# jasonkyuyim/se3_diffusion

Measured on AMD Instinct MI355X. Metric: residues/sec IPA fwd+bwd, higher is better.
Workload: dtype f32

## Files before the change

### include/fd_hip.h

```cpp
#ifndef FD_HIP_H_
#define FD_HIP_H_

#ifdef __cplusplus
extern "C" {
#endif

#define FD_ABI_VERSION 2

const char* fd_last_error(void);
int fd_abi_version(void);
const char* fd_backend(void);
const char* fd_build_flags(void);
long fd_launch_count(void);

typedef struct FdGemmDesc {
  const float* A;
  const float* B;
  float* C;
  int M, N, K;
  long a_rs, a_cs;
  long b_rs, b_cs;
  long ldc;
  int batch, bdiv;
  long a_so, a_si, b_so, b_si, c_so, c_si;
  float alpha;
  int beta;
  const float* bias;
  const float* pair_p;
  const float* pair_q;
  long ld_pair;
  int nres;
  const float* resid;
  long ld_resid;
  const float* gate;
  long ld_gate;
  const float* rowscale;
  int relu;
  int tile;
  int ksplit;
  int mtiles;
  float* a_rowsum;
  const void* b_planes;
  long b_plane_stride;
} FdGemmDesc;

int fd_gemm(const FdGemmDesc* desc, void* stream);
int fd_split_planes(const float* x, long n, void* planes, void* stream);
int fd_gemm_plan(const FdGemmDesc* desc);
int fd_gemm_set_exact_f32(int exact);
int fd_gemm_set_persistent_blocks(int blocks);

int fd_layernorm_fwd(const float* x, long ldx, const float* gamma, const float* beta, const float* rowscale,
                     float* y, long ldy, float* mean, float* rstd, long rows, int C, float eps, void* stream);
int fd_layernorm_bwd(const float* dy, long lddy, const float* x, long ldx, const float* gamma,
                     const float* rowscale, const float* mean, const float* rstd, float* dx, long lddx,
                     int dx_accum, float* dgamma, float* dbeta, long rows, int C, void* stream);
int fd_colsum_acc(const float* X, long ld, long rows, int ncols, float* out, void* stream);
int fd_pair_reduce_acc(const float* X, int nbatch, int n, int C, float* rowsum, float* colsum, long ld_out,
                       void* stream);
int fd_axpby(float* y, const float* x, float a, float b, long n, void* stream);
int fd_add2d(float* dst, long ldd, const float* src, long lds, long rows, int cols, float a, void* stream);
int fd_rowscale(const float* x, long ldx, const float* rs, float* y, long ldy, long rows, int C, void* stream);

#define FD_EDGE_MLP_IMAGE_BYTES (124 * 12288)
int fd_edge_mlp_pack_zb(const float* W40, void* image, void* stream);
int fd_edge_mlp_pack(const float* W1, const float* W2, const float* Wf, long ld, void* image, void* stream);
int fd_edge_mlp_pack_bwd(const float* Wf, const float* W2, const float* W1, long ld, const float* W40, void* image, void* stream);
typedef struct FdEdgeMlpDesc {
  const float* x;
  const void* img;
  const float* p1;
  const float* q1;
  const float* bias2;
  float* save1;
  float* save2;
  const float* pf;
  const float* qf;
  const float* gamma;
  const float* beta;
  const float* rowscale;
  float* y;
  float* mean;
  float* rstd;
  float* out;
  long rows;
  int nres;
  int backward;
  float eps;
  int blocks;
  long ld_pq;
  long ld_pqf;
  float* zb_out;
  const float* zb_bias;
  unsigned* mask1;
  unsigned* mask2;
  const unsigned* gmask1;
  const unsigned* gmask2;
  const float* ln_y;
  const float* ln_mean;
  const float* ln_rstd;
// ... 173 lines not shown
                     float* A, int B, int N, int heads_per_block, void* stream);
#define FD_IPA_FLASH_PART_LD 328
int fd_ipa_flash_fwd_split(const float* proj, const float* zb, const float* qp, const float* kp, const float* vp,
                           const float* head_w, const float* mask, const float* quat, const float* trans, float* feats,
                           float* A, int B, int N, int heads_per_block, int key_splits, float* part, void* stream);

int fd_ipa_flash_bwd(const float* proj, const float* A, const float* zb, const float* dfeats, const float* feats,
                     const float* doptg, const float* ptdot, const float* qp, const float* kp, const float* vp,
                     const float* head_w, const float* trans, float* dL, float* dzb, float* dqp, float* dkp,
                     float* dhead_w, float* hw_part, int B, int N, void* stream);
int fd_ipa_flash_bwd_keys(const float* A, const float* dL, const float* proj, const float* dfeats, const float* doptg,
                          const float* qp, const float* kp, const float* head_w, float* dproj, float* dvp, float* dkp,
                          int B, int N, int heads_per_block, void* stream);
int fd_ipa_opt_bwd_dot(const float* dfeats, const float* feats, const float* quat, const float* trans, float* doptg,
                       float* dframe, float* ptdot, long R, void* stream);

int fd_ipa_dz_acc(const float* dzb, const float* W40, float* dz, long rows, int accumulate, void* stream);

int fd_ipa_kpts_bwd(const float* dL, const float* qp, const float* kp, const float* head_w, float* dkp, int B, int N,
                    void* stream);

int fd_row_softmax_fwd(float* S, const float* key_add, long rows, int N, int rows_per_batch, void* stream);
int fd_row_softmax_bwd(const float* A, float* dA, long rows, int N, void* stream);

int fd_split_rigids(const float* rig7, float scale, const float* t, float tscale, float* quat, float* trans, float* tscaled,
                    long R, int B, void* stream);

int fd_bb_update_fwd(const float* node, long ldn, int cs, const float* dmask, const float* W6, const float* b6,
                     const float* quat, const float* trans, float* upd, float* quat_out, float* trans_out,
                     long R, void* stream);
int fd_bb_update_bwd(const float* dquat_out, const float* dtrans_out, const float* dframe, const float* dmask,
                     const float* upd, const float* quat, float* dquat, float* dtrans, float* dupd, float* dupd_s,
                     long R, void* stream);

typedef struct FdHeadConst {
  float atoms[15];
  float Rd[9];
  float td[3];
  float coord_scale;
  double exp_max_sigma, exp_min_sigma;
  float min_b, max_b;
  int L;
  const double* score_norms;
  const double* omega_grid;
  int n_omega;
} FdHeadConst;
int fd_heads_fwd(const float* rig0, const float* quatF, const float* transF, const float* upsi,
                 const float* gt_psi, long gt_stride, const float* fixed, const float* mask, const float* t,
                 const double* sigma_grid, int ng, const FdHeadConst* c, double* rot_score, float* trans_score,
                 float* rigids, float* psi_out, float* atom37, float* atom14,
                 float* sc_ca_out ,
                 int B, int N, void* stream);
int fd_backbone_atoms(const float* rigids, const float* psi, const FdHeadConst* c, float* atom37, float* atom14,
                      long R, void* stream);
int fd_heads_bwd(const float* rig0, const float* quatF, const float* transF, const float* upsi,
                 const float* psi_out, const float* fixed, const float* mask, const float* t,
                 const double* sigma_grid, int ng, const FdHeadConst* c, const double* d_rot,
                 const float* d_trans_score, const float* d_rigids, const float* d_psi, const float* d_atom37,
                 float* dquatF, float* dtransF, float* dupsi, int B, int N, void* stream);

int fd_igso3_tables(const double* sigma, const double* omega, int ns, int no, int L, double* pdf, double* cdf,
                    double* score_norms, void* stream);
int fd_sample_ref(const double* z_axis, const double* u, const double* z_trans, const double* cdf_row,
                  const double* omega, int no, double coord_scale, float* out, long n, void* stream);
int fd_forward_marginal(const float* rig0, const double* z_axis, const double* u, const double* z_trans,
                        const double* cdf_row, const double* omega, int no,
// ... 100 lines not shown
```

### se3_diffusion_amd/csrc/fd_edge_embed.hip

```cpp
#include "fd_common.h"
#include "../../include/fd_hip.h"

namespace {

#include "fd_chain.h"

constexpr int EE_UNITS = 20;
constexpr int EE_ZB_UNITS = 4;
constexpr int EE_ZB = 40;
constexpr int EE_C = 128;
constexpr float kPi = 3.14159265358979323846f;

__global__ __launch_bounds__(256) void edge_embed_pack_kernel(const float* __restrict__ W0, const float* __restrict__ W2,
                                                              const float* __restrict__ W4, char* __restrict__ img) {
  const int gid = (int)(blockIdx.x * blockDim.x + threadIdx.x);
  if (gid >= EE_UNITS * 4 * 64) return;
  const int lane = gid & 63, i = (gid >> 6) & 3, u = gid >> 8;
  const int m = lane & 15, g = lane >> 4;
  const int layer = u < 4 ? 0 : (u < 12 ? 1 : 2);
  const int r = u - (layer == 0 ? 0 : (layer == 1 ? 4 : 12));
  const int n = 64 * (r & 1) + 16 * i + m, k0 = 32 * (r >> 1);
  float x[8];
#pragma unroll
  for (int e = 0; e < 8; ++e) {
    if (layer == 0) {
      const int k = k0 + 8 * g + e;
      x[e] = k < 54 ? W0[n * 120 + 66 + k] : 0.f;
    } else {
      const int k = k0 + 16 * (e >> 2) + 4 * g + (e & 3);
      x[e] = (layer == 1 ? W2 : W4)[n * EE_C + k];
    }
  }
  uint4 s0, s1, s2;
  em_split8(x, s0, s1, s2);
  char* dst = img + (long)u * EM_UNIT + (i * 3) * EM_PIECE + lane * 16;
  *reinterpret_cast<uint4*>(dst) = s0;
  *reinterpret_cast<uint4*>(dst + EM_PIECE) = s1;
  *reinterpret_cast<uint4*>(dst + 2 * EM_PIECE) = s2;
}

__global__ __launch_bounds__(256) void edge_embed_pack_zb_kernel(const float* __restrict__ W40, char* __restrict__ img) {
  const int gid = (int)(blockIdx.x * blockDim.x + threadIdx.x);
  if (gid >= EE_ZB_UNITS * 4 * 64) return;
  const int lane = gid & 63, i = (gid >> 6) & 3, ks = gid >> 8;
  const int m = lane & 15, g = lane >> 4;
  const int n = 16 * i + m;
  float x[8];
#pragma unroll
  for (int e = 0; e < 8; ++e) {
    const int k = 32 * ks + 16 * (e >> 2) + 4 * g + (e & 3);
    x[e] = n < EE_ZB ? W40[n * EE_C + k] : 0.f;
  }
  uint4 s0, s1, s2;
  em_split8(x, s0, s1, s2);
  char* dst = img + (long)(EE_UNITS + ks) * EM_UNIT + (i * 3) * EM_PIECE + lane * 16;
  *reinterpret_cast<uint4*>(dst) = s0;
  *reinterpret_cast<uint4*>(dst + EM_PIECE) = s1;
  *reinterpret_cast<uint4*>(dst + 2 * EM_PIECE) = s2;
}

template <bool ZB>
__global__ __launch_bounds__(64 * EM_WAVES, 2) void edge_embed_kernel(FdEdgeEmbedDesc d) {
  constexpr int EE_NSTAGE = (EE_UNITS + (ZB ? EE_ZB_UNITS : 0)) / EM_UPS;
  __shared__ __attribute__((aligned(16))) char lds[2 * EM_STAGE];
  const int tid = (int)threadIdx.x;
  const int lane = tid & 63, wave = tid >> 6;
  const int m = lane & 15, g = lane >> 4;
  const long rows = d.rows;
  const long ld_pq = d.ld_pq > 0 ? d.ld_pq : EE_C;
  const int ntiles = (int)((rows + EM_ROWS - 1) / EM_ROWS);
  const int G = (int)gridDim.x, first = (int)blockIdx.x;
  if (first >= ntiles) return;
  const int nmine = (ntiles - first + G - 1) / G;
  const int total_stages = nmine * EE_NSTAGE;

  const char* __restrict__ img_lane = static_cast<const char*>(d.img) + wave * (EM_STAGE / EM_WAVES) + lane * 16;
  char* const lds_wave = lds + wave * (EM_STAGE / EM_WAVES);
  int issued = 0, consumed = 0;
  auto issue_stage = [&]() {
    const char* src = img_lane + (long)(issued % EE_NSTAGE) * EM_STAGE;
    char* dst = lds_wave + (issued & 1) * EM_STAGE;
    fd::glds16x4(src, dst);
    fd::glds16x2(src + 4096, dst + 4096);
    ++issued;
  };
  auto stage_begin = [&]() -> const char* {
    fd::wait_vmem();
    __syncthreads();
    const char* cur = lds + (consumed & 1) * EM_STAGE + lane * 16;
    ++consumed;
    return cur;
// ... 253 lines not shown
```

### se3_diffusion_amd/csrc/fd_edge_embed_bwd.hip

```cpp
#include "fd_common.h"
#include "../../include/fd_hip.h"

namespace {

#include "fd_chain.h"

constexpr int EB_UNITS = 16;
constexpr int EB_NSTAGE = EB_UNITS / EM_UPS;
constexpr int EB_C = 128;

__global__ __launch_bounds__(256) void edge_embed_bwd_pack_kernel(const float* __restrict__ W2, const float* __restrict__ W4,
                                                                  char* __restrict__ img) {
  const int gid = (int)(blockIdx.x * blockDim.x + threadIdx.x);
  if (gid >= EB_UNITS * 4 * 64) return;
  const int lane = gid & 63, i = (gid >> 6) & 3, u = gid >> 8;
  const int m = lane & 15, g = lane >> 4;
  const int layer = u >> 3, r = u & 7;
  const int n = 64 * (r & 1) + 16 * i + m, k0 = 32 * (r >> 1);
  const float* __restrict__ W = layer == 0 ? W4 : W2;
  float x[8];
#pragma unroll
  for (int e = 0; e < 8; ++e) {
    const int k = k0 + 16 * (e >> 2) + 4 * g + (e & 3);
    x[e] = W[k * EB_C + n];
  }
  uint4 s0, s1, s2;
  em_split8(x, s0, s1, s2);
  char* dst = img + (long)u * EM_UNIT + (i * 3) * EM_PIECE + lane * 16;
  *reinterpret_cast<uint4*>(dst) = s0;
  *reinterpret_cast<uint4*>(dst + EM_PIECE) = s1;
  *reinterpret_cast<uint4*>(dst + 2 * EM_PIECE) = s2;
}

__global__ __launch_bounds__(64 * EM_WAVES, 2) void edge_embed_bwd_kernel(FdEdgeEmbedBwdDesc d) {
  __shared__ __attribute__((aligned(16))) char lds[2 * EM_STAGE];
  const int tid = (int)threadIdx.x;
  const int lane = tid & 63, wave = tid >> 6;
  const int m = lane & 15, g = lane >> 4;
  const long rows = d.rows;
  const int ntiles = (int)((rows + EM_ROWS - 1) / EM_ROWS);
  const int G = (int)gridDim.x, first = (int)blockIdx.x;
  if (first >= ntiles) return;
  unsigned* const sched = d.sched;
  const bool dyn = sched != nullptr;
  __shared__ int s_tile;
  const int nmine = (ntiles - first + G - 1) / G;
  const int total_stages = dyn ? 0x7fffffff : nmine * EB_NSTAGE;

  const char* __restrict__ img_lane = static_cast<const char*>(d.img) + wave * (EM_STAGE / EM_WAVES) + lane * 16;
  char* const lds_wave = lds + wave * (EM_STAGE / EM_WAVES);
  int issued = 0, consumed = 0;
  auto issue_stage = [&]() {
    const char* src = img_lane + (long)(issued % EB_NSTAGE) * EM_STAGE;
    char* dst = lds_wave + (issued & 1) * EM_STAGE;
    fd::glds16x4(src, dst);
    fd::glds16x2(src + 4096, dst + 4096);
    ++issued;
  };
  auto stage_begin = [&]() -> const char* {
    fd::wait_vmem();
    __syncthreads();
    const char* cur = lds + (consumed & 1) * EM_STAGE + lane * 16;
    ++consumed;
    return cur;
  };
  auto stage_prefetch = [&]() {
    if (issued < total_stages) issue_stage();
  };
  issue_stage();

  f32x4 dgam[8], dbet[8];
#pragma unroll
  for (int nb = 0; nb < 8; ++nb)
#pragma unroll
    for (int e = 0; e < 4; ++e) dgam[nb][e] = dbet[nb][e] = 0.f;

  int tile = first, nxt = 0;
  for (int ti = 0;;) {
    if (dyn && tid == 0) nxt = G + (int)atomicAdd(&sched[0], 1u);
    const long row = (long)tile * EM_ROWS + wave * 16 + m;
    const bool rok = row < rows;
    const long rc = rok ? row : rows - 1;

    const bool packed = d.gmask2 != nullptr;
    unsigned gm2 = 0u, gm1 = 0u;
    if (packed) {
      gm2 = d.gmask2[rc * 4 + g];
      gm1 = d.gmask1[rc * 4 + g];
    }

    f32x4 d3[8];
    {
      const float rs = (d.rowscale != nullptr ? d.rowscale[rc] : 1.f) * (rok ? 1.f : 0.f);
      const float mean = d.mean[rc], rstd = d.rstd[rc];
      float s1 = 0.f, s2 = 0.f;
#pragma unroll
      for (int nb = 0; nb < 8; ++nb) {
        const int col = 16 * nb + 4 * g;
        const float4 dy = *reinterpret_cast<const float4*>(d.dy + rc * EB_C + col);
        const float4 h = *reinterpret_cast<const float4*>(d.h3 + rc * EB_C + col);
        const float4 gm = *reinterpret_cast<const float4*>(d.gamma + col);
        const float dyv[4] = {dy.x, dy.y, dy.z, dy.w}, hv[4] = {h.x, h.y, h.z, h.w}, gv[4] = {gm.x, gm.y, gm.z, gm.w};
#pragma unroll
        for (int e = 0; e < 4; ++e) {
          const float x = (hv[e] - mean) * rstd;
          const float gy = dyv[e] * rs;
          dgam[nb][e] += gy * x;
          dbet[nb][e] += gy;
          const float t = gy * gv[e];
          d3[nb][e] = t;
          s1 += t;
          s2 += t * x;
// ... 132 lines not shown
    float a = 0.f;
#pragma unroll
    for (int w = 0; w < EM_WAVES; ++w) a += red[(w * 2 + which) * EB_C + col];
    float* dst = which == 0 ? d.dgamma : d.dbeta;
    if (dst != nullptr) atomicAdd(dst + col, a);
  }
}

}

extern "C" int fd_edge_embed_bwd_pack(const float* W2, const float* W4, void* img, void* stream) {
  FD_CHECK_ARG(W2 && W4 && img, "fd_edge_embed_bwd_pack: null operand");
  FD_CHECK_ARG(fd_aligned16(img), "fd_edge_embed_bwd_pack: image must be 16-byte aligned");
  hipLaunchKernelGGL(edge_embed_bwd_pack_kernel, dim3(EB_UNITS * 4 * 64 / 256), dim3(256), 0, (hipStream_t)stream, W2, W4,
                     static_cast<char*>(img));
  FD_CHECK_LAUNCH("fd_edge_embed_bwd_pack");
  return FD_OK;
}

extern "C" int fd_edge_embed_bwd(const FdEdgeEmbedBwdDesc* desc, void* stream) {
  FD_CHECK_ARG(desc != nullptr, "fd_edge_embed_bwd: null descriptor");
  const FdEdgeEmbedBwdDesc& d = *desc;
  FD_CHECK_ARG(d.dy && d.h3 && d.mean && d.rstd && d.gamma && d.img && d.dh3 && d.dh2 && d.dh1,
               "fd_edge_embed_bwd: a required operand is null");
  FD_CHECK_ARG((d.h2 && d.h1) || (d.gmask2 && d.gmask1), "fd_edge_embed_bwd: h2 / h1 or their packed sign masks are required");
  FD_CHECK_ARG(d.rows >= 0, "fd_edge_embed_bwd: negative row count");
  const void* ptrs[] = {d.dy, d.h3, d.gamma, d.h2, d.h1, d.img, d.dh3, d.dh2, d.dh1};
  for (const void* p : ptrs) FD_CHECK_ARG(fd_aligned16(p), "fd_edge_embed_bwd: operands must be 16-byte aligned");
  if (d.rows == 0) return FD_OK;
  const long ntiles = (d.rows + EM_ROWS - 1) / EM_ROWS;
  const int blocks = d.blocks > 0 ? d.blocks : 256 * EM_BLOCKS_PER_CU;
  const long grid = ntiles < blocks ? ntiles : blocks;
  FdEdgeEmbedBwdDesc dd = d;
  if (dd.sched != nullptr && ntiles >= 4 * grid) {
    FD_CHECK_ARG(hipMemsetAsync(dd.sched, 0, sizeof(unsigned), (hipStream_t)stream) == hipSuccess,
                 "fd_edge_embed_bwd: zeroing the tile counter failed");
  } else {
    dd.sched = nullptr;
  }
  hipLaunchKernelGGL(edge_embed_bwd_kernel, dim3((unsigned)grid), dim3(64 * EM_WAVES), 0, (hipStream_t)stream, dd);
  FD_CHECK_LAUNCH("fd_edge_embed_bwd");
  return FD_OK;
}
```

### se3_diffusion_amd/csrc/fd_edge_mlp.hip

```cpp
#if defined(EM_PHASE_TIMING) || defined(EM_ABLATE_PQ) || defined(EM_PLAIN_SAVES)
#include "fd_probe.h"
#endif
#include "fd_common.h"
#include "../../include/fd_hip.h"

#ifdef EM_SHAPE_W8
#define EM_LAUNCH fd_edge_mlp_launch_w8
#else
#define EM_LAUNCH fd_edge_mlp_launch_w4
#endif
int fd_edge_mlp_launch_w4(const FdEdgeMlpDesc& d, hipStream_t st);
int fd_edge_mlp_launch_w8(const FdEdgeMlpDesc& d, hipStream_t st);
int fd_edge_mlp_launch_pair(const FdEdgeMlpDesc& d, hipStream_t st);

namespace {

#include "fd_chain.h"

__device__ __forceinline__ float fd_f4(const float4& v, int e) { return e == 0 ? v.x : e == 1 ? v.y : e == 2 ? v.z : v.w; }

constexpr int EM_UNITS = 120;
constexpr int EM_ZB_UNITS = 4;
constexpr int EM_ZB = 40;
constexpr int EM_RING = 2;
constexpr int EM_H = 384, EM_C = 128;
#ifdef EM_PLAIN_SAVES
#define EM_SAVE4(p, a, b, c, e) (*reinterpret_cast<float4*>(p) = make_float4((a), (b), (c), (e)))
#else
#define EM_SAVE4(p, a, b, c, e) fd::store_nt4((p), (a), (b), (c), (e))
#endif

#ifdef EM_PHASE_TIMING
__device__ unsigned long long em_phase[12];
#define EM_TICK_TO(var)                                                \
  {                                                                    \
    __builtin_amdgcn_sched_barrier(0);                                 \
    const long long t_ = (long long)__builtin_amdgcn_s_memtime();      \
    __builtin_amdgcn_sched_barrier(0);                                 \
    var += t_ - tl_;                                                   \
    tl_ = t_;                                                          \
  }
#define EM_BODY_TO(i) { EM_TICK_TO(tb_); em_add(i, tb_); tb_ = 0; }
#else
#define EM_TICK_TO(var)
#define EM_BODY_TO(i)
#endif

#ifndef EM_SHAPE_W8
struct EmMat {
  const float* p;
  long rs, cs;
};

__global__ __launch_bounds__(256) void edge_mlp_pack16_kernel(EmMat A1, EmMat A2, EmMat A4, char* __restrict__ img, int rot) {
  const int gid = (int)(blockIdx.x * blockDim.x + threadIdx.x);
  if (gid >= EM_UNITS * 4 * 64) return;
  const int lane = gid & 63, i = (gid >> 6) & 3, u = gid >> 8;
  const int m = lane & 15, g = lane >> 4;
  EmMat M;
  int n, k0;
  if (u < 96) {
    const int c = u / 32, r = u % 32, hc = (c + rot) % 3;
    if (r < 8) {
      M = A1; n = 128 * hc + 64 * (r & 1) + 16 * i + m; k0 = 32 * (r >> 1);
    } else {
      const int r2 = r - 8;
      M = A2; n = 64 * (r2 % 6) + 16 * i + m; k0 = 128 * hc + 32 * (r2 / 6);
    }
  } else {
    const int v = u - 96;
    M = A4; n = 64 * (v & 1) + 16 * i + m; k0 = 32 * (v >> 1);
  }
  float x[8];
#pragma unroll
  for (int e = 0; e < 8; ++e) {
    const int k = k0 + 16 * (e >> 2) + 4 * g + (e & 3);
    x[e] = M.p[(long)n * M.rs + (long)k * M.cs];
  }
  uint4 s0, s1, s2;
  em_split8(x, s0, s1, s2);
  char* dst = img + (long)u * EM_UNIT + (i * 3) * EM_PIECE + lane * 16;
  *reinterpret_cast<uint4*>(dst) = s0;
  *reinterpret_cast<uint4*>(dst + EM_PIECE) = s1;
  *reinterpret_cast<uint4*>(dst + 2 * EM_PIECE) = s2;
}

__global__ __launch_bounds__(256) void edge_mlp_pack_zb_kernel(const float* __restrict__ W40, char* __restrict__ img) {
  const int gid = (int)(blockIdx.x * blockDim.x + threadIdx.x);
  if (gid >= EM_ZB_UNITS * 4 * 64) return;
  const int lane = gid & 63, i = (gid >> 6) & 3, ks = gid >> 8;
  const int m = lane & 15, g = lane >> 4;
  const int n = 16 * i + m;
  float x[8];
#pragma unroll
  for (int e = 0; e < 8; ++e) {
    const int k = 32 * ks + 16 * (e >> 2) + 4 * g + (e & 3);
    x[e] = n < EM_ZB ? W40[n * EM_C + k] : 0.f;
  }
  uint4 s0, s1, s2;
  em_split8(x, s0, s1, s2);
  char* dst = img + (long)(EM_UNITS + ks) * EM_UNIT + (i * 3) * EM_PIECE + lane * 16;
  *reinterpret_cast<uint4*>(dst) = s0;
  *reinterpret_cast<uint4*>(dst + EM_PIECE) = s1;
  *reinterpret_cast<uint4*>(dst + 2 * EM_PIECE) = s2;
}

__global__ __launch_bounds__(256) void edge_mlp_pack_zbw_kernel(const float* __restrict__ W40, char* __restrict__ img) {
  const int gid = (int)(blockIdx.x * blockDim.x + threadIdx.x);
  if (gid >= EM_ZB_UNITS * 4 * 64) return;
  const int lane = gid & 63, i = (gid >> 6) & 3, u = gid >> 8;
  const int m = lane & 15, g = lane >> 4;
  const int n = 64 * (u & 1) + 16 * i + m, k0 = 32 * (u >> 1);
  float x[8];
#pragma unroll
  for (int e = 0; e < 8; ++e) {
    const int k = k0 + 8 * g + e;
    x[e] = k < EM_ZB ? W40[k * EM_C + n] : 0.f;
  }
  uint4 s0, s1, s2;
  em_split8(x, s0, s1, s2);
  char* dst = img + (long)u * EM_UNIT + (i * 3) * EM_PIECE + lane * 16;
  *reinterpret_cast<uint4*>(dst) = s0;
  *reinterpret_cast<uint4*>(dst + EM_PIECE) = s1;
  *reinterpret_cast<uint4*>(dst + 2 * EM_PIECE) = s2;
}

#endif

template <bool BWD, bool ZB = false, bool TRAIN = false, bool LNB = false, bool ZBW = false>
__global__ __launch_bounds__(64 * EM_WAVES, 2) void edge_mlp16_kernel(FdEdgeMlpDesc d) {
  static_assert(!BWD || (!ZB && TRAIN), "backward: no zb layer, always with the saves");
  static_assert(BWD || (!LNB && !ZBW), "the fused prologue is a backward option");
  constexpr int EM_NSTAGE = (EM_UNITS + (ZB ? EM_ZB_UNITS : 0) + (ZBW ? EM_ZB_UNITS : 0)) / EM_UPS;
  __shared__ __attribute__((aligned(16))) char lds[EM_RING * EM_STAGE];
  __shared__ float lnacc[LNB ? 2 * EM_C : 1];
  const int tid = (int)threadIdx.x;
  const int lane = tid & 63, wave = tid >> 6;
  const int m = lane & 15, g = lane >> 4;
  const long rows = d.rows;
#ifdef EM_PHASE_TIMING
  long long p0_ = 0, p1_ = 0, p2_ = 0, p3_ = 0, p4_ = 0, p5_ = 0, p6_ = 0, p7_ = 0, p8_ = 0, p9_ = 0;
  long long tb_ = 0, tl_ = (long long)__builtin_amdgcn_s_memtime();
  auto em_add = [&](int i, long long v) {
    switch (i) {
      case 0: p0_ += v; break;
      case 2: p2_ += v; break;
      case 3: p3_ += v; break;
      case 4: p4_ += v; break;
      case 5: p5_ += v; break;
      case 6: p6_ += v; break;
      case 7: p7_ += v; break;
      case 8: p8_ += v; break;
      default: p9_ += v; break;
    }
  };
#endif
  const long ld_pq = d.ld_pq > 0 ? d.ld_pq : EM_H, ld_pqf = d.ld_pqf > 0 ? d.ld_pqf : EM_C;
// ... 10 lines not shown
  char* const lds_wave = lds + wave * (EM_STAGE / EM_WAVES);
  int issued = 0, consumed = 0;
  auto issue_stage = [&]() __attribute__((always_inline)) {
    const char* src = img_lane + (long)(issued % EM_NSTAGE) * EM_STAGE;
    char* dst = lds_wave + (issued % EM_RING) * EM_STAGE;
    if (EM_PPW == 6) {
      fd::glds16x4(src, dst);
      fd::glds16x2(src + 4096, dst + 4096);
    } else {
      fd::glds16x3(src, dst);
    }
    ++issued;
  };
  auto stage_begin = [&]() __attribute__((always_inline)) -> const char* {
    EM_TICK_TO(tb_);
    fd::wait_vmem();
    __syncthreads();
    EM_TICK_TO(p1_);
    const char* cur = lds + (consumed % EM_RING) * EM_STAGE + lane * 16;
    ++consumed;
    return cur;
  };
  auto stage_prefetch = [&]() __attribute__((always_inline)) {
    if (issued < total_stages) issue_stage();
  };
  issue_stage();
  if (LNB) {
    if (tid < 2 * EM_C) lnacc[tid] = 0.f;
    __syncthreads();
  }

  int tile = first, nxt = 0;
  for (int ti = 0;;) {
    if (dyn && tid == 0) nxt = G + (int)atomicAdd(&sched[0], 1u);
    const long row = (long)tile * EM_ROWS + wave * 16 + m;
    const bool rok = row < rows;
    const long rc = rok ? row : rows - 1;
    const long qi = rc / d.nres;
    const long qj = (qi / d.nres) * d.nres + (rc - qi * d.nres);

    f32x4 X[BWD ? 8 : 1], Xk[2][2];
    auto load_xk = [&](int buf, int ks) __attribute__((always_inline)) {
#pragma unroll
      for (int i = 0; i < 2; ++i) {
        const float4 v = *reinterpret_cast<const float4*>(d.x + rc * EM_C + 16 * (2 * ks + i) + 4 * g);
        Xk[buf][i][0] = v.x; Xk[buf][i][1] = v.y; Xk[buf][i][2] = v.z; Xk[buf][i][3] = v.w;
      }
    };
    if (BWD) {
#pragma unroll
      for (int nb = 0; nb < 8; ++nb) {
        float4 v = make_float4(0.f, 0.f, 0.f, 0.f);
        if (!LNB || d.x != nullptr) v = *reinterpret_cast<const float4*>(d.x + rc * EM_C + 16 * nb + 4 * g);
        X[nb][0] = v.x; X[nb][1] = v.y; X[nb][2] = v.z; X[nb][3] = v.w;
      }
    } else {
      load_xk(0, 0);
    }
    if (LNB) {
      if (ZBW) {
        float kz[2][8];
        {
          const float* zp = d.dzb + rc * EM_ZB + 8 * g;
          const float4 v = *reinterpret_cast<const float4*>(zp);
          const float4 w = *reinterpret_cast<const float4*>(zp + 4);
          kz[0][0] = v.x; kz[0][1] = v.y; kz[0][2] = v.z; kz[0][3] = v.w;
          kz[0][4] = w.x; kz[0][5] = w.y; kz[0][6] = w.z; kz[0][7] = w.w;
// ... 343 lines not shown
  }
  if (tid == 0) __hip_atomic_fetch_add(&em_phase[10], 1ull, __ATOMIC_RELAXED, __HIP_MEMORY_SCOPE_AGENT);
#endif
  if (dyn) fd::wait_vmem();
  if (LNB) {
    __syncthreads();
    if (tid < EM_C) {
      if (d.ln_dgamma != nullptr) atomicAdd(d.ln_dgamma + tid, lnacc[tid]);
    } else if (tid < 2 * EM_C) {
      if (d.ln_dbeta != nullptr) atomicAdd(d.ln_dbeta + (tid - EM_C), lnacc[tid]);
    }
  }
}

}

#ifdef EM_PHASE_TIMING
extern "C" int fd_edge_mlp_phases(unsigned long long* host12, int reset) {
  if (host12 != nullptr && hipMemcpyFromSymbol(host12, HIP_SYMBOL(em_phase), sizeof(em_phase)) != hipSuccess) return -1;
  if (reset) {
    unsigned long long z[12] = {0};
    if (hipMemcpyToSymbol(HIP_SYMBOL(em_phase), z, sizeof(z)) != hipSuccess) return -1;
  }
  return 0;
}
#endif

int EM_LAUNCH(const FdEdgeMlpDesc& d, hipStream_t st) {
  const long ntiles = (d.rows + EM_ROWS - 1) / EM_ROWS;
  const int blocks = d.blocks > 0 ? d.blocks : 256 * EM_BLOCKS_PER_CU;
  const int grid = (int)(ntiles < blocks ? ntiles : blocks);
  const dim3 g3(grid), b3(64 * EM_WAVES);
  FdEdgeMlpDesc dd = d;
  if (dd.sched != nullptr && ntiles >= 4L * grid) {
    FD_CHECK_ARG(hipMemsetAsync(dd.sched, 0, sizeof(unsigned), st) == hipSuccess, "fd_edge_mlp: zeroing the tile counter failed");
  } else {
    dd.sched = nullptr;
  }
  const bool zbv = d.zb_out != nullptr, train = d.save1 != nullptr;
#define EM_GO(...) hipLaunchKernelGGL(HIP_KERNEL_NAME(edge_mlp16_kernel<__VA_ARGS__>), g3, b3, 0, st, dd)
  if (d.backward) {
    if (d.ln_y != nullptr && d.dzb != nullptr) EM_GO(true, false, true, true, true);
    else if (d.ln_y != nullptr) EM_GO(true, false, true, true, false);
    else EM_GO(true, false, true, false, false);
  } else if (zbv) {
    if (train) EM_GO(false, true, true); else EM_GO(false, true, false);
  } else {
    if (train) EM_GO(false, false, true); else EM_GO(false, false, false);
  }
#undef EM_GO
  FD_CHECK_LAUNCH("fd_edge_mlp");
  return FD_OK;
}

#ifndef EM_SHAPE_W8
extern "C" int fd_edge_mlp_pack(const float* W1, const float* W2, const float* Wf, long ld, void* img, void* stream) {
  FD_CHECK_ARG(W1 && W2 && Wf && img, "fd_edge_mlp_pack: null operand");
  FD_CHECK_ARG(fd_aligned16(img), "fd_edge_mlp_pack: image must be 16-byte aligned");
  EmMat m1{W1, ld, 1}, m2{W2, ld, 1}, m4{Wf, ld, 1};
  hipLaunchKernelGGL(edge_mlp_pack16_kernel, dim3(EM_UNITS * 4 * 64 / 256), dim3(256), 0, (hipStream_t)stream, m1, m2, m4,
                     static_cast<char*>(img), 0);
  FD_CHECK_LAUNCH("fd_edge_mlp_pack");
  return FD_OK;
}

extern "C" int fd_edge_mlp_pack_bwd(const float* Wf, const float* W2, const float* W1, long ld, const float* W40, void* img,
                                    void* stream) {
  FD_CHECK_ARG(Wf && W2 && W1 && img, "fd_edge_mlp_pack_bwd: null operand");
  FD_CHECK_ARG(fd_aligned16(img), "fd_edge_mlp_pack_bwd: image must be 16-byte aligned");
  char* base = static_cast<char*>(img);
  if (W40 != nullptr) {
    hipLaunchKernelGGL(edge_mlp_pack_zbw_kernel, dim3(EM_ZB_UNITS * 4 * 64 / 256), dim3(256), 0, (hipStream_t)stream, W40, base);
    base += (long)EM_ZB_UNITS * EM_UNIT;
  }
  EmMat m1{Wf, 1, ld}, m2{W2, 1, ld}, m4{W1, 1, ld};
  hipLaunchKernelGGL(edge_mlp_pack16_kernel, dim3(EM_UNITS * 4 * 64 / 256), dim3(256), 0, (hipStream_t)stream, m1, m2, m4, base, 1);
  FD_CHECK_LAUNCH("fd_edge_mlp_pack_bwd");
  return FD_OK;
}

extern "C" int fd_edge_mlp_pack_zb(const float* W40, void* img, void* stream) {
  FD_CHECK_ARG(W40 && img, "fd_edge_mlp_pack_zb: null operand");
  FD_CHECK_ARG(fd_aligned16(img), "fd_edge_mlp_pack_zb: image must be 16-byte aligned");
  hipLaunchKernelGGL(edge_mlp_pack_zb_kernel, dim3(EM_ZB_UNITS * 4 * 64 / 256), dim3(256), 0, (hipStream_t)stream, W40,
                     static_cast<char*>(img));
  FD_CHECK_LAUNCH("fd_edge_mlp_pack_zb");
  return FD_OK;
}

extern "C" int fd_edge_mlp(const FdEdgeMlpDesc* desc, void* stream) {
  FD_CHECK_ARG(desc != nullptr, "fd_edge_mlp: null descriptor");
  const FdEdgeMlpDesc& d = *desc;
  FD_CHECK_ARG(d.img && d.out && (d.x || (d.backward && d.ln_y && d.dzb)), "fd_edge_mlp: x / img / out are required");
  FD_CHECK_ARG(d.ln_y == nullptr || (d.backward && d.ln_mean && d.ln_rstd && d.ln_gamma),
               "fd_edge_mlp: the fused LayerNorm backward (ln_y) is a backward option and needs ln_mean / ln_rstd / ln_gamma");
  FD_CHECK_ARG(d.dzb == nullptr || d.ln_y != nullptr, "fd_edge_mlp: dzb needs the fused LayerNorm-backward prologue (ln_y)");
  FD_CHECK_ARG(d.nres > 0 && d.rows >= 0, "fd_edge_mlp: bad extents");
  if (d.backward) {
    FD_CHECK_ARG(d.gmask1 && d.gmask2 && d.save1 && d.save2,
                 "fd_edge_mlp(backward): the packed sign masks of h2 (gmask1) and h1 (gmask2) and the outputs d2 (save1) / d1 (save2) "
                 "are required");
    FD_CHECK_ARG(!d.mask1 && !d.mask2 && !d.zb_out, "fd_edge_mlp(backward): mask1 / mask2 / zb_out are forward outputs");
  } else {
    FD_CHECK_ARG(d.p1 && d.q1 && d.bias2 && d.pf && d.qf && d.gamma && d.beta,
                 "fd_edge_mlp(forward): p1 / q1 / bias2 / pf / qf / gamma / beta are required");
    const int nsave = (d.save1 != nullptr) + (d.save2 != nullptr) + (d.mask1 != nullptr) + (d.mask2 != nullptr);
    FD_CHECK_ARG(nsave == 0 || nsave == 4,
                 "fd_edge_mlp(forward): the training outputs save1 (h1), save2 (h2 + [z | 0 | 0]), mask1, mask2 come together");
    FD_CHECK_ARG(nsave == 4 || (!d.y && !d.mean && !d.rstd), "fd_edge_mlp(forward): y / mean / rstd are training outputs (with the saves)");
    FD_CHECK_ARG(!d.gmask1 && !d.gmask2, "fd_edge_mlp(forward): gmask1 / gmask2 are backward inputs");
  }
  const void* ptrs[] = {d.x, d.img, d.out, d.p1, d.q1, d.bias2, d.save1, d.save2, d.pf, d.qf,
                        d.gamma, d.beta, d.y, d.ln_y, d.ln_gamma, d.dy_out, d.dzb};
  for (const void* p : ptrs) FD_CHECK_ARG(fd_aligned16(p), "fd_edge_mlp: operands must be 16-byte aligned");
  if (d.rows == 0) return FD_OK;
  FD_CHECK_ARG(d.zb_out == nullptr || (fd_aligned16(d.zb_out) && fd_aligned16(d.zb_bias)),
               "fd_edge_mlp: zb_out / zb_bias must be 16-byte aligned (the image must carry the fd_edge_mlp_pack_zb units)");
  FD_CHECK_ARG(d.shape == 0 || d.shape == 2 || d.shape == 4 || d.shape == 8,
               "fd_edge_mlp: shape is 0 (by size), 2 (two waves per 16 rows: inference forward), 4 or 8 (waves per block)");
// ... 10 lines not shown
```

### se3_diffusion_amd/csrc/fd_frames.hip

```cpp
#include "fd_common.h"
#include "../../include/fd_hip.h"

namespace {

struct Rot { float r[9]; };

__device__ __forceinline__ Rot quat_to_rot(const float* __restrict__ q) {
  const float a = q[0], b = q[1], c = q[2], d = q[3];
  Rot R;
  R.r[0] = a * a + b * b - c * c - d * d;
  R.r[1] = 2.f * (b * c - a * d);
  R.r[2] = 2.f * (b * d + a * c);
  R.r[3] = 2.f * (b * c + a * d);
  R.r[4] = a * a - b * b + c * c - d * d;
  R.r[5] = 2.f * (c * d - a * b);
  R.r[6] = 2.f * (b * d - a * c);
  R.r[7] = 2.f * (c * d + a * b);
  R.r[8] = a * a - b * b - c * c + d * d;
  return R;
}

__device__ __forceinline__ void rot_grad_to_quat(const float* __restrict__ q, const float* G, float* dq) {
  const float a = q[0], b = q[1], c = q[2], d = q[3];
  dq[0] += 2.f * a * (G[0] + G[4] + G[8]) + 2.f * (-d * G[1] + c * G[2] + d * G[3] - b * G[5] - c * G[6] + b * G[7]);
// ... 108 lines not shown
    const float gw = d * dn0, gx = d * dn1, gy = d * dn2, gz = d * dn3;
    float dq[4];
    dq[0] = dn0 + (vx * gx + vy * gy + vz * gz);
    dq[1] = dn1 + (-vx * gw - vz * gy + vy * gz);
    dq[2] = dn2 + (-vy * gw + vz * gx - vx * gz);
    dq[3] = dn3 + (-vz * gw - vy * gx + vx * gy);
    float du[6];
    du[0] = -x * gw + w * gx + z * gy - y * gz;
    du[1] = -y * gw - z * gx + w * gy + x * gz;
    du[2] = -z * gw + y * gx - x * gy + w * gz;
    const Rot R = quat_to_rot(q);
    const float* gt = dtrans_out + r * 3;
    const float t0 = gt[0] * d, t1 = gt[1] * d, t2 = gt[2] * d;
    du[3] = R.r[0] * t0 + R.r[3] * t1 + R.r[6] * t2;
    du[4] = R.r[1] * t0 + R.r[4] * t1 + R.r[7] * t2;
    du[5] = R.r[2] * t0 + R.r[5] * t1 + R.r[8] * t2;
    float G[9];
    G[0] = t0 * u[3]; G[1] = t0 * u[4]; G[2] = t0 * u[5];
    G[3] = t1 * u[3]; G[4] = t1 * u[4]; G[5] = t1 * u[5];
    G[6] = t2 * u[3]; G[7] = t2 * u[4]; G[8] = t2 * u[5];
    float dt0 = gt[0], dt1 = gt[1], dt2 = gt[2];
    if (dframe) {
      const float* f = dframe + r * 12;
#pragma unroll
      for (int k = 0; k < 9; ++k) G[k] += f[k];
      dt0 += f[9]; dt1 += f[10]; dt2 += f[11];
    }
    rot_grad_to_quat(q, G, dq);
#pragma unroll
    for (int k = 0; k < 4; ++k) dquat[r * 4 + k] = dq[k];
    dtrans[r * 3 + 0] = dt0; dtrans[r * 3 + 1] = dt1; dtrans[r * 3 + 2] = dt2;
#pragma unroll
    for (int k = 0; k < 6; ++k) { dupd[r * 6 + k] = du[k]; dupd_s[r * 6 + k] = du[k] * d; }
  }
}

constexpr double kDirichletOmega = 1e-2;

__device__ __forceinline__ void igso3_series_small(double om, double sg, int L, double* f, double* df, double* d2f) {
  const double so = sin(om), co = cos(om);
  double s = 0.0, c = 1.0;
  const double q = exp(-sg * sg);
  double w = 1.0, r = q;
  double R0 = 1.0, R1 = 0.0, R2 = 0.0;
  double F = 0.0, D = 0.0, D2 = 0.0;
  for (int l = 0; l < L; ++l) {
    if (l > 0) {
      const double s2 = s * co + c * so;
      c = c * co - s * so;
      s = s2;
      const double k = (double)l;
      R0 += 2.0 * c;
      R1 -= 2.0 * k * s;
      R2 -= 2.0 * k * k * c;
    }
    const double cw = (double)(2 * l + 1) * w;
    F += cw * R0;
    D += cw * R1;
    D2 += cw * R2;
    w *= r;
    r *= q;
    if (w == 0.0) break;
  }
  *f = F; *df = D; *d2f = D2;
}

// ... 350 lines not shown
  FD_CHECK_LAUNCH("fd_row_softmax_fwd");
  return FD_OK;
}

extern "C" int fd_row_softmax_bwd(const float* A, float* dA, long rows, int N, void* stream) {
  if (rows == 0 || N == 0) return FD_OK;
  hipLaunchKernelGGL(row_softmax_bwd_kernel, dim3(rows4_grid(rows, 16384)), dim3(256), 0, (hipStream_t)stream, A, dA,
                     rows, N);
  FD_CHECK_LAUNCH("fd_row_softmax_bwd");
  return FD_OK;
}

extern "C" int fd_bb_update_fwd(const float* node, long ldn, int cs, const float* dmask, const float* W6,
                                const float* b6, const float* quat, const float* trans, float* upd, float* quat_out,
                                float* trans_out, long R_, void* stream) {
  if (R_ == 0) return FD_OK;
  hipLaunchKernelGGL(bb_update_fwd_kernel, dim3(rows4_grid(R_, 8192)), dim3(256), 0, (hipStream_t)stream, node, ldn,
                     cs, dmask, W6, b6, quat, trans, upd, quat_out, trans_out, R_);
  FD_CHECK_LAUNCH("fd_bb_update_fwd");
  return FD_OK;
}

extern "C" int fd_bb_update_bwd(const float* dquat_out, const float* dtrans_out, const float* dframe,
                                const float* dmask, const float* upd, const float* quat, float* dquat, float* dtrans,
                                float* dupd, float* dupd_s, long R_, void* stream) {
  if (R_ == 0) return FD_OK;
  long g = (R_ + 255) / 256;
  hipLaunchKernelGGL(bb_update_bwd_kernel, dim3((unsigned)(g > 4096 ? 4096 : g)), dim3(256), 0, (hipStream_t)stream,
                     dquat_out, dtrans_out, dframe, dmask, upd, quat, dquat, dtrans, dupd, dupd_s, R_);
  FD_CHECK_LAUNCH("fd_bb_update_bwd");
  return FD_OK;
}

static HeadConst make_hc(const FdHeadConst* c) {
  HeadConst hc;
  for (int i = 0; i < 15; ++i) hc.atoms[i] = c->atoms[i];
  for (int i = 0; i < 9; ++i) hc.Rd[i] = c->Rd[i];
  for (int i = 0; i < 3; ++i) hc.td[i] = c->td[i];
  hc.coord_scale = c->coord_scale;
  hc.exp_max_sigma = c->exp_max_sigma;
  hc.exp_min_sigma = c->exp_min_sigma;
  hc.min_b = c->min_b;
  hc.max_b = c->max_b;
  hc.L = c->L;
  hc.score_norms = c->score_norms;
  hc.omega_grid = c->omega_grid;
  hc.n_omega = c->n_omega;
  return hc;
}

extern "C" int fd_heads_fwd(const float* rig0, const float* quatF, const float* transF, const float* upsi,
                            const float* gt_psi, long gt_stride, const float* fixed, const float* mask,
                            const float* t, const double* sigma_grid, int ng, const FdHeadConst* c,
                            double* rot_score, float* trans_score, float* rigids, float* psi_out, float* atom37,
                            float* atom14, float* sc_ca_out, int B, int N, void* stream) {
  FD_CHECK_ARG(c != nullptr, "fd_heads_fwd: null constants");
  FD_CHECK_ARG(!c->score_norms || (c->omega_grid && c->n_omega > 1), "fd_heads_fwd: cached score table without its grid");
  const long R_ = (long)B * N;
  if (R_ == 0) return FD_OK;
  long g = (R_ + 127) / 128;
  hipLaunchKernelGGL(heads_fwd_kernel, dim3((unsigned)(g > 8192 ? 8192 : g)), dim3(128), 0, (hipStream_t)stream, rig0,
                     quatF, transF, upsi, gt_psi, gt_stride, fixed, mask, t, sigma_grid, ng, make_hc(c), rot_score,
                     trans_score, rigids, psi_out, atom37, atom14, sc_ca_out, N, R_);
  FD_CHECK_LAUNCH("fd_heads_fwd");
  return FD_OK;
}
// ... 19 lines not shown
```

### se3_diffusion_amd/csrc/fd_norm.hip

```cpp
#include "fd_common.h"
#include "../../include/fd_hip.h"

namespace {

constexpr int MAXC_PER_LANE = 8;

__global__ __launch_bounds__(256) void layernorm_fwd_kernel(
    const float* __restrict__ x, long ldx, const float* __restrict__ gamma, const float* __restrict__ beta,
    const float* __restrict__ rowscale, float* __restrict__ y, long ldy, float* __restrict__ mean_out,
    float* __restrict__ rstd_out, long rows, int C, float eps) {
  const int lane = fd::lane_id(), wave = fd::wave_id();
  const int npl = C / 64;
  for (long row = (long)blockIdx.x * 4 + wave; row < rows; row += (long)gridDim.x * 4) {
    const float* xr = x + row * ldx;
    float v[MAXC_PER_LANE], gm[MAXC_PER_LANE], bt[MAXC_PER_LANE];
    float s = 0.f;
#pragma unroll
    for (int k = 0; k < MAXC_PER_LANE; ++k)
      if (k < npl) { v[k] = xr[lane + 64 * k]; s += v[k]; }
    const float rs = rowscale ? rowscale[row] : 1.f;
#pragma unroll
    for (int k = 0; k < MAXC_PER_LANE; ++k)
      if (k < npl) { gm[k] = gamma[lane + 64 * k]; bt[k] = beta[lane + 64 * k]; }
    const float mean = fd::wave_sum(s) / (float)C;
// ... 43 lines not shown
        xh[k] = (xr[c] - m) * r;
        g[k] = d * gamma[c];
        ag[k] += d * xh[k];
        ab[k] += d;
        s1 += g[k];
        s2 += g[k] * xh[k];
      }
    s1 = fd::wave_sum(s1) / (float)C;
    s2 = fd::wave_sum(s2) / (float)C;
    float* dxr = dx + row * lddx;
#pragma unroll
    for (int k = 0; k < MAXC_PER_LANE; ++k)
      if (k < npl) {
        int c = lane + 64 * k;
        float v = r * (g[k] - s1 - xh[k] * s2);
        dxr[c] = dx_accum ? dxr[c] + v : v;
      }
  }
  if (dgamma) {
#pragma unroll
    for (int k = 0; k < MAXC_PER_LANE; ++k)
      if (k < npl) { red[0][wave][lane + 64 * k] = ag[k]; red[1][wave][lane + 64 * k] = ab[k]; }
    __syncthreads();
    for (int c = (int)threadIdx.x; c < C; c += 256) {
      float a = red[0][0][c] + red[0][1][c] + red[0][2][c] + red[0][3][c];
      float b = red[1][0][c] + red[1][1][c] + red[1][2][c] + red[1][3][c];
      atomicAdd(&dgamma[c], a);
      atomicAdd(&dbeta[c], b);
    }
  }
}

constexpr int LNB_U = 4;
template <int NCH>
__global__ __launch_bounds__(256) void layernorm_bwd4_kernel(
    const float* __restrict__ dy, long lddy, const float* __restrict__ x, long ldx,
    const float* __restrict__ gamma, const float* __restrict__ rowscale, const float* __restrict__ mean,
    const float* __restrict__ rstd, float* __restrict__ dx, long lddx, int dx_accum,
    float* __restrict__ dgamma, float* __restrict__ dbeta, long rows, int C) {
  __shared__ float red[2][4][512];
  const int lane = fd::lane_id(), wave = fd::wave_id();
  int col[NCH];
  bool cok[NCH];
  float4 gm[NCH], ag[NCH], ab[NCH];
#pragma unroll
  for (int k = 0; k < NCH; ++k) {
    col[k] = 4 * (lane + 64 * k);
    cok[k] = col[k] < C;
    if (!cok[k]) col[k] = 0;
    gm[k] = *reinterpret_cast<const float4*>(gamma + col[k]);
    ag[k] = make_float4(0.f, 0.f, 0.f, 0.f);
    ab[k] = ag[k];
  }
  const float invc = 1.0f / (float)C;
  const long wslot = (long)blockIdx.x * 4 + wave, nwaves = (long)gridDim.x * 4;
  for (long base = wslot * LNB_U; base < rows; base += nwaves * LNB_U) {
    float4 xv[LNB_U][NCH], dv[LNB_U][NCH], old[LNB_U][NCH];
    float m[LNB_U], rr[LNB_U], rs[LNB_U];
#pragma unroll
    for (int u = 0; u < LNB_U; ++u) {
      const long r = base + u < rows ? base + u : rows - 1;
#pragma unroll
      for (int k = 0; k < NCH; ++k) {
        xv[u][k] = *reinterpret_cast<const float4*>(x + r * ldx + col[k]);
        dv[u][k] = *reinterpret_cast<const float4*>(dy + r * lddy + col[k]);
        if (dx_accum) old[u][k] = *reinterpret_cast<const float4*>(dx + r * lddx + col[k]);
      }
      m[u] = mean[r];
      rr[u] = rstd[r];
      rs[u] = rowscale ? rowscale[r] : 1.f;
    }
    float4 xh[LNB_U][NCH], g[LNB_U][NCH];
    float s1[LNB_U], s2[LNB_U];
#pragma unroll
    for (int u = 0; u < LNB_U; ++u) {
      const bool ok = base + u < rows;
      s1[u] = 0.f;
      s2[u] = 0.f;
#pragma unroll
      for (int k = 0; k < NCH; ++k) {
        const float sc = (ok && cok[k]) ? rs[u] : 0.f;
        const float4 d = make_float4(dv[u][k].x * sc, dv[u][k].y * sc, dv[u][k].z * sc, dv[u][k].w * sc);
        xh[u][k] = make_float4((xv[u][k].x - m[u]) * rr[u], (xv[u][k].y - m[u]) * rr[u], (xv[u][k].z - m[u]) * rr[u],
                               (xv[u][k].w - m[u]) * rr[u]);
        g[u][k] = make_float4(d.x * gm[k].x, d.y * gm[k].y, d.z * gm[k].z, d.w * gm[k].w);
        ag[k].x += d.x * xh[u][k].x; ag[k].y += d.y * xh[u][k].y; ag[k].z += d.z * xh[u][k].z; ag[k].w += d.w * xh[u][k].w;
        ab[k].x += d.x; ab[k].y += d.y; ab[k].z += d.z; ab[k].w += d.w;
        s1[u] += (g[u][k].x + g[u][k].y) + (g[u][k].z + g[u][k].w);
        s2[u] += (g[u][k].x * xh[u][k].x + g[u][k].y * xh[u][k].y) + (g[u][k].z * xh[u][k].z + g[u][k].w * xh[u][k].w);
      }
    }
#pragma unroll
    for (int u = 0; u < LNB_U; ++u) {
      s1[u] = fd::wave_sum(s1[u]) * invc;
      s2[u] = fd::wave_sum(s2[u]) * invc;
    }
#pragma unroll
    for (int u = 0; u < LNB_U; ++u) {
      if (base + u >= rows) continue;
#pragma unroll
      for (int k = 0; k < NCH; ++k) {
        if (!cok[k]) continue;
        float4 o;
        o.x = rr[u] * (g[u][k].x - s1[u] - xh[u][k].x * s2[u]);
        o.y = rr[u] * (g[u][k].y - s1[u] - xh[u][k].y * s2[u]);
        o.z = rr[u] * (g[u][k].z - s1[u] - xh[u][k].z * s2[u]);
        o.w = rr[u] * (g[u][k].w - s1[u] - xh[u][k].w * s2[u]);
        if (dx_accum) { o.x += old[u][k].x; o.y += old[u][k].y; o.z += old[u][k].z; o.w += old[u][k].w; }
        *reinterpret_cast<float4*>(dx + (base + u) * lddx + col[k]) = o;
      }
    }
  }
  if (dgamma) {
#pragma unroll
    for (int k = 0; k < NCH; ++k)
      if (cok[k]) {
        *reinterpret_cast<float4*>(&red[0][wave][col[k]]) = ag[k];
        *reinterpret_cast<float4*>(&red[1][wave][col[k]]) = ab[k];
      }
    __syncthreads();
    for (int c = (int)threadIdx.x; c < C; c += 256) {
      float a = red[0][0][c] + red[0][1][c] + red[0][2][c] + red[0][3][c];
      float b = red[1][0][c] + red[1][1][c] + red[1][2][c] + red[1][3][c];
      atomicAdd(&dgamma[c], a);
      atomicAdd(&dbeta[c], b);
    }
  }
}

constexpr int LN_U = 4;

__device__ __forceinline__ float half_wave_sum(float v) {
#pragma unroll
  for (int o = 16; o > 0; o >>= 1) v += __shfl_xor(v, o);
  return v;
}

__global__ __launch_bounds__(256) void layernorm_fwd128_kernel(
    const float* __restrict__ x, long ldx, const float* __restrict__ gamma, const float* __restrict__ beta,
    const float* __restrict__ rowscale, float* __restrict__ y, long ldy, float* __restrict__ mean_out,
    float* __restrict__ rstd_out, long rows, float eps) {
  const int lane = fd::lane_id(), wave = fd::wave_id();
// ... 295 lines not shown
  if (rows == 0) return FD_OK;
  if (C == 128 && ln128_ok(x, ldx) && ln128_ok(y, ldy) && fd_aligned16(gamma) && fd_aligned16(beta)) {
    long g = (rows + 8 * LN_U - 1) / (8 * LN_U);
    int grid = (int)(g < 1 ? 1 : (g > 4096 ? 4096 : g));
    hipLaunchKernelGGL(layernorm_fwd128_kernel, dim3(grid), dim3(256), 0, (hipStream_t)stream, x, ldx, gamma, beta,
                       rowscale, y, ldy, mean, rstd, rows, eps);
    FD_CHECK_LAUNCH("fd_layernorm_fwd(128)");
    return FD_OK;
  }
  hipLaunchKernelGGL(layernorm_fwd_kernel, dim3(ln_grid(rows)), dim3(256), 0, (hipStream_t)stream, x, ldx, gamma,
                     beta, rowscale, y, ldy, mean, rstd, rows, C, eps);
  FD_CHECK_LAUNCH("fd_layernorm_fwd");
  return FD_OK;
}

extern "C" int fd_layernorm_bwd(const float* dy, long lddy, const float* x, long ldx, const float* gamma,
                                const float* rowscale, const float* mean, const float* rstd, float* dx, long lddx,
                                int dx_accum, float* dgamma, float* dbeta, long rows, int C, void* stream) {
  FD_CHECK_ARG(C % 64 == 0 && C <= 64 * MAXC_PER_LANE, "fd_layernorm_bwd: C=%d must be a multiple of 64 <= 512", C);
  FD_CHECK_ARG((dgamma == nullptr) == (dbeta == nullptr), "fd_layernorm_bwd: dgamma/dbeta come together");
  if (rows == 0) return FD_OK;
  if (C == 128 && ln128_ok(x, ldx) && ln128_ok(dy, lddy) && ln128_ok(dx, lddx) && fd_aligned16(gamma)) {
    long g128 = (rows + 8 * LN_U - 1) / (8 * LN_U);
    int grid128 = (int)(g128 < 1 ? 1 : (g128 > 512 ? 512 : g128));
    hipLaunchKernelGGL(layernorm_bwd128_kernel, dim3(grid128), dim3(256), 0, (hipStream_t)stream, dy, lddy, x, ldx,
                       gamma, rowscale, mean, rstd, dx, lddx, dx_accum, dgamma, dbeta, rows);
    FD_CHECK_LAUNCH("fd_layernorm_bwd(128)");
    return FD_OK;
  }
  long g = (rows + 15) / 16;
  int grid = (int)(g < 1 ? 1 : (g > 1024 ? 1024 : g));
  if (ln128_ok(x, ldx) && ln128_ok(dy, lddy) && ln128_ok(dx, lddx) && fd_aligned16(gamma)) {
    if (C <= 256)
      hipLaunchKernelGGL(layernorm_bwd4_kernel<1>, dim3(grid), dim3(256), 0, (hipStream_t)stream, dy, lddy, x, ldx, gamma,
                         rowscale, mean, rstd, dx, lddx, dx_accum, dgamma, dbeta, rows, C);
    else
      hipLaunchKernelGGL(layernorm_bwd4_kernel<2>, dim3(grid), dim3(256), 0, (hipStream_t)stream, dy, lddy, x, ldx, gamma,
                         rowscale, mean, rstd, dx, lddx, dx_accum, dgamma, dbeta, rows, C);
    FD_CHECK_LAUNCH("fd_layernorm_bwd(x4)");
    return FD_OK;
  }
  hipLaunchKernelGGL(layernorm_bwd_kernel, dim3(grid), dim3(256), 0, (hipStream_t)stream, dy, lddy, x, ldx, gamma,
                     rowscale, mean, rstd, dx, lddx, dx_accum, dgamma, dbeta, rows, C);
  FD_CHECK_LAUNCH("fd_layernorm_bwd");
  return FD_OK;
}

extern "C" int fd_colsum_acc(const float* X, long ld, long rows, int ncols, float* out, void* stream) {
  if (rows == 0 || ncols == 0) return FD_OK;
  long g = (rows + 15) / 16;
  int grid = (int)(g < 1 ? 1 : (g > 1024 ? 1024 : g));
  if ((ld & 3) == 0 && (ncols & 3) == 0 && fd_aligned16(X)) {
    hipLaunchKernelGGL(colsum4_kernel, dim3(grid), dim3(256), 0, (hipStream_t)stream, X, ld, rows, ncols, out);
    FD_CHECK_LAUNCH("fd_colsum_acc");
    return FD_OK;
  }
  hipLaunchKernelGGL(colsum_kernel, dim3(grid), dim3(256), 0, (hipStream_t)stream, X, ld, rows, ncols, out);
  FD_CHECK_LAUNCH("fd_colsum_acc");
  return FD_OK;
}

extern "C" int fd_pair_reduce_acc(const float* X, int nbatch, int n, int C, float* rowsum, float* colsum,
                                  long ld_out, void* stream) {
  if (nbatch == 0 || n == 0) return FD_OK;
  if (rowsum && colsum && (C % PR_C) == 0 && fd_aligned16(X)) {
    const int nich = fd_cdiv(n, PR_I), ncc = C / PR_C;
    hipLaunchKernelGGL(pair_reduce2_kernel, dim3(nbatch * nich * ncc, fd_cdiv(n, PR_J)), dim3(256), 0, (hipStream_t)stream,
                       X, n, C, rowsum, colsum, ld_out, nich, ncc);
    FD_CHECK_LAUNCH("fd_pair_reduce_acc(fused)");
    return FD_OK;
  }
  int threads = C >= 256 ? 256 : (C >= 128 ? 128 : 64);
  if (rowsum) {
    hipLaunchKernelGGL(pair_reduce_kernel, dim3(nbatch * n), dim3(threads), 0, (hipStream_t)stream, X, n, C, rowsum,
                       (float*)nullptr, ld_out);
    FD_CHECK_LAUNCH("fd_pair_reduce_acc(row)");
  }
// ... 37 lines not shown
```

### se3_diffusion_amd/hip.py

```python
from __future__ import annotations

import ctypes
import os
from ctypes import POINTER, Structure, c_char_p, c_double, c_float, c_int, c_long, c_void_p

import torch

_HERE = os.path.dirname(os.path.abspath(__file__))
LIB_PATH = os.path.join(_HERE, "lib", "libfd_hip.so")


_RAW_STREAM = getattr(torch._C, "_cuda_getCurrentRawStream", None)


class FdError(RuntimeError):
    pass


class FdGemmDesc(Structure):
    _fields_ = [
        ("A", c_void_p), ("B", c_void_p), ("C", c_void_p),
        ("M", c_int), ("N", c_int), ("K", c_int),
        ("a_rs", c_long), ("a_cs", c_long),
        ("b_rs", c_long), ("b_cs", c_long),
# ... 60 lines not shown

EDGE_MLP_W8_MIN_ROWS = 65536
EDGE_MLP_PAIR_MAX_ROWS = 16384
EDGE_MLP_IMAGE_BYTES = 124 * 12288


class FdEdgeEmbedDesc(Structure):
    __slots__ = ()
    _fields_ = [
        ("seq_idx", c_void_p), ("sc_ca", c_void_p), ("idenom", c_void_p), ("dg_lower", c_void_p), ("dg_upper", c_void_p),
        ("img", c_void_p), ("p", c_void_p), ("q", c_void_p), ("bias2", c_void_p), ("bias3", c_void_p),
        ("gamma", c_void_p), ("beta", c_void_p), ("rowscale", c_void_p),
        ("h1", c_void_p), ("h2", c_void_p), ("h3", c_void_p), ("mean", c_void_p), ("rstd", c_void_p), ("out", c_void_p),
        ("rows", c_long), ("nres", c_int), ("eps", c_float), ("blocks", c_int), ("zb_out", c_void_p), ("zb_bias", c_void_p),
        ("mask1", c_void_p), ("mask2", c_void_p), ("ld_pq", c_long),
    ]


EDGE_EMBED_IMAGE_BYTES = 24 * 12288


class FdEdgeEmbedBwdDesc(Structure):
    __slots__ = ()
    _fields_ = [
        ("dy", c_void_p), ("h3", c_void_p), ("mean", c_void_p), ("rstd", c_void_p), ("gamma", c_void_p), ("rowscale", c_void_p),
        ("h2", c_void_p), ("h1", c_void_p), ("img", c_void_p), ("dh3", c_void_p), ("dh2", c_void_p), ("dh1", c_void_p),
        ("dgamma", c_void_p), ("dbeta", c_void_p), ("rows", c_long), ("blocks", c_int), ("gmask2", c_void_p), ("gmask1", c_void_p),
        ("sched", c_void_p),
    ]


EDGE_EMBED_BWD_IMAGE_BYTES = 16 * 12288

class FdLnGemmDesc(Structure):
    __slots__ = ()
    _fields_ = [
        ("x", c_void_p), ("ldx", c_long), ("gamma", c_void_p), ("beta", c_void_p), ("ln_rowscale", c_void_p),
        ("ln_out", c_void_p), ("ld_ln_out", c_long), ("W", c_void_p), ("ldw", c_long), ("bias", c_void_p),
        ("resid", c_void_p), ("ld_resid", c_long), ("out", c_void_p), ("ldo", c_long),
        ("M", c_int), ("N", c_int), ("K", c_int), ("relu", c_int), ("eps", c_float), ("ln_cols", c_int),
    ]


PAIR_DW_MAX_ITEMS = 8


class FdPairDwItem(Structure):
    __slots__ = ()
    _fields_ = [
        ("A", c_void_p), ("lda", c_long), ("A_add", c_void_p), ("ld_add", c_long), ("B", c_void_p), ("ldb", c_long),
        ("C", c_void_p), ("ldc", c_long), ("a_colsum", c_void_p), ("trans", c_int), ("a_bands", c_int), ("b_cols", c_int),
    ]


class FdPairDwDesc(Structure):
    _fields_ = [("item", FdPairDwItem * PAIR_DW_MAX_ITEMS), ("nitems", c_int), ("rows", c_long), ("blocks", c_int)]


GROUP_DW_MAX_ITEMS = 32


class FdGroupDwItem(Structure):
    __slots__ = ()
    _fields_ = [("A", c_void_p), ("B", c_void_p), ("C", c_void_p), ("a_colsum", c_void_p),
                ("lda", c_int), ("ldb", c_int), ("ldc", c_int), ("n_out", c_int), ("k_in", c_int)]

# ... 22 lines not shown


def _ptr(t, off=0):
    if t is None:
        return None
    if isinstance(t, tuple):
        t, off = t
    return t.data_ptr() + t.element_size() * int(off)


def fill_ptrs(desc, **fields):
    tens = []
    for name, t in fields.items():
        if t is None:
            continue
        if type(t) is tuple:
            off = t[1]
            t = t[0]
            setattr(desc, name, t.data_ptr() + t.element_size() * int(off))
        else:
            setattr(desc, name, t.data_ptr())
        tens.append(t)
    return tens


_SIGS = {
    "fd_gemm": "Ss",
    "fd_gemm_plan": "S",
    "fd_split_planes": "plps",
    "fd_gemm_set_exact_f32": "i",
    "fd_gemm_set_persistent_blocks": "i",
    "fd_edge_mlp_pack": "ppplps",
    "fd_edge_mlp": "Ss",
    "fd_edge_mlp_pack_zb": "pps",
    "fd_edge_mlp_pack_bwd": "ppplpps",
    "fd_edge_embed_pack": "pppps",
    "fd_edge_embed": "Ss",
    "fd_edge_embed_pack_zb": "pps",
    "fd_edge_embed_bwd_pack": "ppps",
    "fd_edge_embed_bwd": "Ss",
    "fd_ln_gemm": "Ss",
    "fd_pair_dw": "Ss",
    "fd_group_dw": "Ss",
    "fd_layernorm_fwd": "plpppplpplifs",
    "fd_layernorm_bwd": "plplpppppl" + "ipplis",
    "fd_colsum_acc": "pllips",
    "fd_pair_reduce_acc": "piiippls",
    "fd_axpby": "ppffls",
    "fd_rowscale": "plppllis",
    "fd_add2d": "plpllifs",
    "fd_node_feats": "ppppppiis",
    "fd_node_feats_ld": "ppppppliis",
    "fd_edge_feats": "pppppppppiis",
    "fd_ipa_points_fwd": "pppppppiliiiis",
    "fd_ipa_points_bwd": "pppppppliiiis",
    "fd_ipa_softmax_fwd": "ppppppiis",
    "fd_ipa_attn_fwd": "ppppppppiis",
    "fd_ipa_flash_fwd": "ppppppppppp" + "iiis",
    "fd_ipa_flash_fwd_split": "ppppppppppp" + "iiii" + "ps",
    "fd_ipa_flash_bwd": "pppppppppppp" + "pppppp" + "iis",
    "fd_ipa_flash_bwd_keys": "pppppppp" + "ppp" + "iiis",
    "fd_ipa_opt_bwd_dot": "ppppppp" + "ls",
    "fd_seq_attn_fwd": "ppppfiis",
    "fd_seq_attn_bwd": "pppppfiis",
    "fd_ipa_attn_bwd": "pppppppppppppiis",
    "fd_ipa_softmax_bwd": "ppppppppppiis",
    "fd_ipa_kpts_bwd": "pppppiis",
    "fd_ipa_dz_acc": "ppplis",
    "fd_ipa_opt_fwd": "ppppls",
    "fd_ipa_opt_bwd": "pppppls",
    "fd_ipa_opair_fwd": "pppiis",
    "fd_ipa_opair_bwd": "pppppiis",
    "fd_row_softmax_fwd": "pplii" + "s",
    "fd_row_softmax_bwd": "pplis",
    "fd_split_rigids": "pfpfppplis",
    "fd_bb_update_fwd": "plipppppppp" + "ls",
    "fd_bb_update_bwd": "pppppppppp" + "ls",
    "fd_heads_fwd": "pppp" + "pl" + "ppp" + "pi" + "S" + "ppppppp" + "iis",
    "fd_heads_bwd": "ppppp" + "ppp" + "pi" + "S" + "ppppp" + "ppp" + "iis",
    "fd_backbone_atoms": "ppSppls",
    "fd_igso3_tables": "ppiiippps",
    "fd_sample_ref": "pppppidpls",
    "fd_forward_marginal": "ppppppipdddipppp" + "ls",
    "fd_forward_marginal_batch": "ppppppippdipppp" + "iis",
    "fd_se3_reverse_step": "ppppppiiddpdddiiips",
    "fd_se3_reverse_step_f32": "ppppppiiddpdddiiips",
    "fd_se3_reverse_step_net": "ppppppiiddpdddiiips",
    "fd_sample_advance": "ppppilpipps",
    "fd_sample_record": "ppppp" + "S" + "piili" + "pppp" + "s",
    "fd_dsm_loss": "Ss",
    "fd_adam_step": "pppplffffffs",
    "fd_adam_step_ema": "ppppplfffffffs",
    "fd_grad_stats": "plpps",
    "fd_adam_step_guarded": "pppplddddd" + "i" + "pp" + "s",
    "fd_adam_step_guarded_ema": "ppppplddddd" + "i" + "pp" + "di" + "s",
    "fd_backbone_metrics": "plpiips",
    "fd_aligned_rmsd": "plplpppiipps",
    "fd_tm_search": "plplppp" + "iiiii" + "ppp" + "s",
}
_CT = {"p": c_void_p, "i": c_int, "l": c_long, "f": c_float, "d": c_double, "S": c_void_p, "s": c_void_p}


class FdLib:

    def __init__(self, path: str):
        if not os.path.exists(path):
            raise FdError(
                f"HIP extension not found at {path}. Build it with "
                f"`python -m se3_diffusion_amd.build` (hipcc, gfx950). There is no CPU fallback.")
        self.path = path
# ... 138 lines not shown
```

### se3_diffusion_amd/network.py

```python
from __future__ import annotations

import math

import torch

from . import hip, ops
from .ops import empty, zeros, mv, lib
from .options import opts

H, C, PQ, PV, CZ4 = 8, 256, 8, 12, 32
CS, CZ = 256, 128
LDP = 6816
LDF = 2688
ZB = 40
TD, TH, THD = 320, 4, 80


def check_conf(conf):
    ipa = conf.ipa
    want = dict(c_s=256, c_z=128, c_hidden=256, c_skip=64, no_heads=8, no_qk_points=8, no_v_points=12,
                seq_tfmr_num_heads=4)
    for k, v in want.items():
        if getattr(ipa, k) != v:
            raise NotImplementedError(
# ... 2 lines not shown
        raise NotImplementedError("node_embed_size/edge_embed_size must be 256/128")
    if int(getattr(ipa, "seq_tfmr_num_layers", 2)) < 1:
        raise NotImplementedError(f"model.ipa.seq_tfmr_num_layers={ipa.seq_tfmr_num_layers}: at least one transformer layer per block")
    e = conf.embed
    if e.index_embed_size != 32 or e.num_bins != 22 or not e.embed_self_conditioning:
        raise NotImplementedError("embed config must match config/base.yaml (index 32, 22 bins, self-conditioning)")


def _lin_grads(G, wname, bname, dy, x, M, N, K, w_off=0, w_ld=None):
    if G is None:
        return
    db = G[bname] if (bname is not None and bname in G) else None
    if wname in G:
        W = G[wname]
        if ops.queue_dw(dy, x, (W, w_off, w_ld if w_ld is not None else W.shape[1]), M, N, K, db=db):
            return
        ops.side(lambda: ops.linear_dw(dy, x, (W, w_off, w_ld if w_ld is not None else W.shape[1]), M, N, K, db=db),
                 (dy[0], x[0]), M)
    elif db is not None:
        ops.side(lambda: ops.bias_grad(dy, db, M, N), (dy[0],), M)


def mlp3_ln_fwd(P, pre, x, M, K0, Cc, rowscale, W0=None):
    dev = x[0]
    h1 = empty((M, Cc), dev); h2 = empty((M, Cc), dev); h3 = empty((M, Cc), dev); y = empty((M, Cc), dev)
    mean = empty((M,), dev); rstd = empty((M,), dev)
    ops.linear(x, mv(P[f"{pre}.0.weight"] if W0 is None else W0), P[f"{pre}.0.bias"], mv(h1), M, Cc, K0, relu=True)
    ops.linear(mv(h1), mv(P[f"{pre}.2.weight"]), P[f"{pre}.2.bias"], mv(h2), M, Cc, Cc, relu=True)
    ops.linear(mv(h2), mv(P[f"{pre}.4.weight"]), P[f"{pre}.4.bias"], mv(h3), M, Cc, Cc)
    ops.layernorm(mv(h3), P[f"{pre}.5.weight"], P[f"{pre}.5.bias"], mv(y), M, Cc, rowscale=rowscale, save=(mean, rstd))
    return y, dict(x=x, h1=h1, h2=h2, h3=h3, mean=mean, rstd=rstd, rowscale=rowscale, M=M, K0=K0, C=Cc)


def mlp3_ln_bwd(P, G, pre, sv, dy):
    M, K0, Cc = sv["M"], sv["K0"], sv["C"]
    dev = dy
    dh3 = empty((M, Cc), dev)
    ops.layernorm_bwd(mv(dy), mv(sv["h3"]), P[f"{pre}.5.weight"], sv["mean"], sv["rstd"], mv(dh3), M, Cc,
                      rowscale=sv["rowscale"], dgamma=G[f"{pre}.5.weight"], dbeta=G[f"{pre}.5.bias"])
    _lin_grads(G, f"{pre}.4.weight", f"{pre}.4.bias", mv(dh3), mv(sv["h2"]), M, Cc, Cc)
    dh2 = empty((M, Cc), dev)
    ops.linear_dx(mv(dh3), mv(P[f"{pre}.4.weight"]), mv(dh2), M, Cc, Cc, gate=mv(sv["h2"]))
    _lin_grads(G, f"{pre}.2.weight", f"{pre}.2.bias", mv(dh2), mv(sv["h1"]), M, Cc, Cc)
    dh1 = empty((M, Cc), dev)
    ops.linear_dx(mv(dh2), mv(P[f"{pre}.2.weight"]), mv(dh1), M, Cc, Cc, gate=mv(sv["h1"]))
    _lin_grads(G, f"{pre}.0.weight", f"{pre}.0.bias", mv(dh1), sv["x"], M, Cc, K0)


def fused_embed():
    return opts.fused_embed and not lib().exact_f32


def embed_fwd(P, feats, B, N, cache=None, save=True, zb_next=None):
    dev = feats["res_mask"]
    mask = feats["res_mask"]
    tfreq, idenom, lower, upper = ops.feature_tables(dev.device)
    tscaled = feats["tscaled"] if "tscaled" in feats else (feats["t"] * 10000).float().contiguous()
    fixed = feats["fixed_mask"]
    seq = feats["seq_idx"]
    R, Pn = B * N, B * N * N
    pre = "embedding_layer.edge_embedder"
    padded = cache is not None and not save and opts.embed_first_padded and fused_embed()
    NFL = 72 if padded else 65
    nf = empty((R, NFL), dev)
    if padded:
        lib().call("fd_node_feats_ld", seq, tscaled, fixed, tfreq, idenom, nf, NFL, B, N)
        if "embed_first" not in cache:
            Wn, W0e = P["embedding_layer.node_embedder.0.weight"], P[f"{pre}.0.weight"]
            Wn72 = torch.zeros((CS, NFL), device=Wn.device); Wn72[:, :65] = Wn
            Wpq = torch.zeros((2 * CZ, NFL), device=Wn.device); Wpq[:CZ, :33] = W0e[:, :33]; Wpq[CZ:, :33] = W0e[:, 33:66]
            bpq = torch.cat([P[f"{pre}.0.bias"], torch.zeros_like(P[f"{pre}.0.bias"])]).contiguous()
            cache["embed_first"] = (Wn72, Wpq, bpq)
        Wn72, Wpq, bpq = cache["embed_first"]
        node, sv_n = mlp3_ln_fwd(P, "embedding_layer.node_embedder", mv(nf), R, NFL, CS, mask, W0=Wn72)
    else:
        lib().call("fd_node_feats", seq, tscaled, fixed, tfreq, idenom, nf, B, N)
        node, sv_n = mlp3_ln_fwd(P, "embedding_layer.node_embedder", mv(nf), R, 65, CS, mask)
    emask = pair_mask(mask, B, N) if cache is None else cache.setdefault("emask", None)
    if emask is None:
        emask = cache["emask"] = pair_mask(mask, B, N)
    if not fused_embed():
        ef = empty((Pn, 120), dev)
        lib().call("fd_edge_feats", seq, tscaled, fixed, feats["sc_ca_t"], tfreq, idenom, lower, upper, ef, B, N)
        edge, sv_e = mlp3_ln_fwd(P, pre, mv(ef), Pn, 120, CZ, emask)
        return node, edge, dict(node=sv_n, edge=sv_e, emask=emask), None
    W0 = P[f"{pre}.0.weight"]
    ld_pq = 0
    if padded:
        pq = empty((R, 2 * CZ), dev)
        ops.linear(mv(nf), mv(Wpq), bpq, mv(pq), R, 2 * CZ, NFL)
        p_, q_, ld_pq = pq, pq[:, CZ:], 2 * CZ
    else:
        p_ = empty((R, CZ), dev); q_ = empty((R, CZ), dev)
        ops.linear((nf, 0, 65), (W0, 0, 120), P[f"{pre}.0.bias"], mv(p_), R, CZ, 33)
        ops.linear((nf, 0, 65), (W0, 33, 120), None, mv(q_), R, CZ, 33)
    use_zb = (opts.zb_from_edge and zb_next is not None and zb_next[0].is_contiguous() and zb_next[0].data_ptr() % 16 == 0
              and zb_next[1].data_ptr() % 16 == 0)
    key = ("ee_img", pre, use_zb)
    if cache is not None and key in cache:
        img = cache[key]
    else:
        img = ops.edge_embed_pack(W0, P[f"{pre}.2.weight"], P[f"{pre}.4.weight"], W40=zb_next[0] if use_zb else None)
        if cache is not None:
            cache[key] = img
    edge = empty((Pn, CZ), dev)
    kw = {}
    zb = None
    if use_zb:
        zb = empty((Pn, ZB), dev)
        kw.update(zb_out=zb, zb_bias=zb_next[1])
    if save:
        h1 = empty((Pn, CZ), dev); h2 = empty((Pn, CZ), dev); h3 = empty((Pn, CZ), dev)
        mean = empty((Pn,), dev); rstd = empty((Pn,), dev)
        kw.update(h1=h1, h2=h2, h3=h3, mean=mean, rstd=rstd)
        if opts.packed_gates:
            mh1 = empty((Pn, 4), dev, torch.int32); mh2 = empty((Pn, 4), dev, torch.int32)
            kw.update(mask1=mh1, mask2=mh2)
    ops.edge_embed(seq, feats["sc_ca_t"], idenom, lower, upper, img, p_, q_, P[f"{pre}.2.bias"], P[f"{pre}.4.bias"],
                   P[f"{pre}.5.weight"], P[f"{pre}.5.bias"], edge, Pn, N, rowscale=emask, ld_pq=ld_pq, **kw)
    sv_e = None
    if save:
        sv_e = dict(x=None, h1=h1, h2=h2, h3=h3, mean=mean, rstd=rstd, rowscale=emask, M=Pn, K0=120, C=CZ,
                    mh1=kw.get("mask1"), mh2=kw.get("mask2"),
                    regen=(seq, tscaled, fixed, feats["sc_ca_t"], B, N))
    return node, edge, dict(node=sv_n, edge=sv_e, emask=emask), zb


def embed_regen_early(sv, G):
    se = sv["edge"]
    if G is None or se is None or se.get("x") is not None or "regen" not in se:
        return
    seq, tscaled, fixed, sc, B, N = se["regen"]
    Pn = B * N * N
    if not ops.side_active(sc, Pn):
        return
    tfreq, idenom, lower, upper = ops.feature_tables(sc.device)
    ef = empty((Pn, 120), sc)
    ops.side(lambda: lib().call("fd_edge_feats", seq, tscaled, fixed, sc, tfreq, idenom, lower, upper, ef, B, N), (ef,), Pn)
    se["x_early"] = ef


def embed_bwd(P, G, sv, dnode, dedge):
    mlp3_ln_bwd(P, G, "embedding_layer.node_embedder", sv["node"], dnode)
    se = sv["edge"]
    if se.get("x_early") is not None:
        se = dict(se, x=mv(se.pop("x_early")))
    if se.get("x") is None:
        seq, tscaled, fixed, sc, B, N = se["regen"]
        tfreq, idenom, lower, upper = ops.feature_tables(dedge.device)
        ef = empty((B * N * N, 120), dedge)
        lib().call("fd_edge_feats", seq, tscaled, fixed, sc, tfreq, idenom, lower, upper, ef, B, N)
        se = dict(se, x=mv(ef))
    pre = "embedding_layer.edge_embedder"
    if (opts.fused_embed_bwd and fused_embed() and G is not None and se.get("regen") is not None
            and all(f"{pre}.{l}.{t}" in G for l in (0, 2, 4) for t in ("weight", "bias"))):
        M = se["M"]
        dh3 = empty((M, CZ), dedge); dh2 = empty((M, CZ), dedge); dh1 = empty((M, CZ), dedge)
        img = ops.edge_embed_bwd_pack(P[f"{pre}.2.weight"], P[f"{pre}.4.weight"])
        ops.edge_embed_bwd(dedge, se["h3"], se["mean"], se["rstd"], P[f"{pre}.5.weight"], se["rowscale"], se["h2"], se["h1"], img,
                           dh3, dh2, dh1, G[f"{pre}.5.weight"], G[f"{pre}.5.bias"], M, gmask2=se.get("mh2"), gmask1=se.get("mh1"))
        x = se["x"]
        items = [(mv(dh3), mv(se["h2"]), mv(G[f"{pre}.4.weight"]), G[f"{pre}.4.bias"], CZ, CZ),
                 (mv(dh2), mv(se["h1"]), mv(G[f"{pre}.2.weight"]), G[f"{pre}.2.bias"], CZ, CZ),
                 (mv(dh1), x, mv(G[f"{pre}.0.weight"]), G[f"{pre}.0.bias"], CZ, se["K0"])]
        ops.side(lambda: ops.group_dw(items, M), (dh3, dh2, dh1, se["h2"], se["h1"], x[0]), M)
        return
    mlp3_ln_bwd(P, G, pre, se, dedge)


def pair_mask(mask, B, N):
    em = empty((B * N * N,), mask)
    src = mask.reshape(B, 1, N).expand(B, N, N).contiguous()
    lib().call("fd_rowscale", src, N, mask.reshape(-1), em, N, B * N, N)
    return em


def _adjacent_view(a, b, shape, *more):
    ts = (a, b) + more
    for x, y in zip(ts[:-1], ts[1:]):
        if not (x.is_contiguous() and y.is_contiguous() and x.dtype == y.dtype and x.device == y.device
                and x.untyped_storage().data_ptr() == y.untyped_storage().data_ptr()
                and x.storage_offset() + x.numel() == y.storage_offset()):
            return None
    if a.data_ptr() % 16 != 0:
        return None
    strides, st = [], 1
    for d in reversed(shape):
        strides.append(st)
        st *= d
    return a.detach().as_strided(shape, tuple(reversed(strides)))

# ... 67 lines not shown
        A = empty((B, H, N, N), dev) if train else None
        if split > 1:
            part = empty((split * R * H * 328,), dev)
            L.call("fd_ipa_flash_fwd_split", proj, zb, qp, kp, vp, P[f"{pre}.head_weights"], mask, quat, trans, feats, None, B, N,
                   opts.flash_ipa_hpb or 4, split, part)
        else:
            L.call("fd_ipa_flash_fwd", proj, zb, qp, kp, vp, P[f"{pre}.head_weights"], mask, quat, trans, feats, A, B, N,
                   opts.flash_ipa_hpb)
    else:
        A = empty((B, H, N, N), dev)
        L.gemm(proj, proj, A, N, N, C, (LDP, 1), (1, LDP), N, b_off=2048, batch=B * H, bdiv=H,
               a_bs=(N * LDP, C), b_bs=(N * LDP, 2 * C), c_bs=(H * N * N, N * N), alpha=math.sqrt(1.0 / (3 * C)))
        if fused_attn:
            L.call("fd_ipa_attn_fwd", A, zb, qp, kp, kpT, P[f"{pre}.head_weights"], mask, feats, B, N)
        else:
            L.call("fd_ipa_softmax_fwd", A, zb, qp, kp, P[f"{pre}.head_weights"], mask, B, N)
        optg = empty((R, H, PV * 3), dev)
        L.gemm(A, vp, optg, N, PV * 3, N, (N, 1), (H * PV * 3, 1), H * PV * 3, batch=B * H, bdiv=H,
               a_bs=(H * N * N, N * N), b_bs=(N * H * PV * 3, PV * 3), c_bs=(N * H * PV * 3, PV * 3))
        L.call("fd_ipa_opt_fwd", optg, quat, trans, feats, R)
        L.gemm(A, proj, feats, N, C, N, (N, 1), (LDP, 1), LDF, b_off=2048 + C, batch=B * H, bdiv=H,
               a_bs=(H * N * N, N * N), b_bs=(N * LDP, 2 * C), c_bs=(N * LDF, C))
        if not fused_attn:
            L.call("fd_ipa_opair_fwd", A, zb, feats, B, N)
    x1 = empty((R, CS), dev) if out_view is None else out_view[0]
    ops.linear(mv(feats), mv(P[f"{pre}.linear_out.weight"]), P[f"{pre}.linear_out.bias"], mv(x1) if out_view is None else out_view,
               R, CS, LDF, rowscale=mask, resid=s)
    ops.STATS["ipa_flash_fwd" if flash else "ipa_sequence_fwd"] += 1
    sv = dict(s=s, z=z, quat=quat, trans=trans, mask=mask, proj=proj, qp=qp, kp=kp, kpT=kpT, vp=vp, W40=W40, b40=b40, zb=zb, A=A,
              feats=feats, B=B, N=N, fused_attn=fused_attn, flash_bwd=flash_bwd)
    return x1, sv


def ipa_bwd(P, G, pre, sv, dx1, ds, dz, dframe, dz_accumulate=True, defer_dz=False):
    B, N = sv["B"], sv["N"]
    R, Pn = B * N, B * N * N
    dev = dx1
    L = lib()
    mask = sv["mask"]
    s, z, proj, A, feats, zb = sv["s"], sv["z"], sv["proj"], sv["A"], sv["feats"], sv["zb"]
    quat, qp, kp, vp = sv["quat"], sv["qp"], sv["kp"], sv["vp"]
    dm = empty((R, CS), dev)
    L.call("fd_rowscale", dx1, CS, mask, dm, CS, R, CS)
    ops.add_view(ds, mv(dx1), R, CS)
    _lin_grads(G, f"{pre}.linear_out.weight", f"{pre}.linear_out.bias", mv(dm), mv(feats), R, CS, LDF)
    dfeats = empty((R, LDF), dev)
    ops.linear_dx(mv(dm), mv(P[f"{pre}.linear_out.weight"]), mv(dfeats), R, CS, LDF)
    dproj = empty((R, LDP), dev)
    dqp = empty((R, H, PQ * 3), dev); dkp = empty((R, H, PQ * 3), dev)
    dhw = G[f"{pre}.head_weights"] if G is not None else zeros((H,), dev)
    hw_part = empty((R, H), dev)
    dzb = empty((Pn, ZB), dev)
    doptg = empty((R, H, PV * 3), dev)
    flash = sv["flash_bwd"]
    ops.STATS["ipa_flash_bwd" if flash else "ipa_sequence_bwd"] += 1
    if flash:
        ptdot = empty((R, H), dev)
        L.call("fd_ipa_opt_bwd_dot", dfeats, feats, quat, sv["trans"], doptg, dframe, ptdot, R)
        dA = empty((B, H, N, N), dev)
        keys = bool(opts.flash_ipa_keys and N <= opts.flash_ipa_keys_max_n)
        L.call("fd_ipa_flash_bwd", proj, A, zb, dfeats, feats, doptg, ptdot, qp, kp, vp, P[f"{pre}.head_weights"], sv["trans"],
               dA, dzb, dqp, None if keys else dkp, dhw, hw_part, B, N)
    else:
        dA = empty((B, H, N, N), dev)
        L.gemm(dfeats, proj, dA, N, N, C, (LDF, 1), (1, LDP), N, b_off=2048 + C, batch=B * H, bdiv=H,
               a_bs=(N * LDF, C), b_bs=(N * LDP, 2 * C), c_bs=(H * N * N, N * N))
        L.call("fd_ipa_opt_bwd", dfeats, feats, quat, doptg, dframe, R)
        L.gemm(doptg, vp, dA, N, N, PV * 3, (H * PV * 3, 1), (1, H * PV * 3), N, batch=B * H, bdiv=H,
               a_bs=(N * H * PV * 3, PV * 3), b_bs=(N * H * PV * 3, PV * 3), c_bs=(H * N * N, N * N), beta=True)
        if sv["fused_attn"]:
            L.call("fd_ipa_attn_bwd", A, dA, zb, dfeats, qp, kp, sv["kpT"], P[f"{pre}.head_weights"], dzb, dqp, dkp, dhw,
                   hw_part, B, N)
        else:
            L.call("fd_ipa_opair_bwd", A, zb, dfeats, dA, dzb, B, N)
            L.call("fd_ipa_softmax_bwd", A, dA, qp, kp, P[f"{pre}.head_weights"], dzb, dqp, dkp, dhw, hw_part, B, N)
    dvp = empty((R, H, PV * 3), dev)
    sc = math.sqrt(1.0 / (3 * C))
# ... 26 lines not shown
                ops.linear_dw(mv(dzb), mv(z), mv(gW), Pn, ZB, CZ)
                ops.bias_grad(mv(dzb), gb, Pn, ZB)
            ops.side(_grads_zb, (dzb, z), Pn)
        else:
            dW40 = zeros((ZB, CZ), dev); db40 = zeros((ZB,), dev)
            ops.linear_dw(mv(dzb), mv(z), mv(dW40), Pn, ZB, CZ)
            ops.bias_grad(mv(dzb), db40, Pn, ZB)
            G[f"{pre}.linear_b.weight"] += dW40[:H]; G[f"{pre}.down_z.weight"] += dW40[H:]
            G[f"{pre}.linear_b.bias"] += db40[:H]; G[f"{pre}.down_z.bias"] += db40[H:]
    pv = _proj_views(P, pre)
    gv = _proj_views(G, pre) if G is not None else None
    if pv is not None and gv is not None:
        ops.linear_dx(mv(dproj), mv(pv[0]), ds, R, LDP, CS, beta=True)
        if not ops.queue_dw(mv(dproj), s, mv(gv[0]), R, LDP, CS, db=gv[1]):
            ops.side(lambda: ops.linear_dw(mv(dproj), s, mv(gv[0]), R, LDP, CS, db=gv[1]), (dproj, s[0]), R)
        return (dzb, sv["W40"]) if defer_dz else None
    for name, off, n in (("linear_q", 0, 2048), ("linear_kv", 2048, 4096), ("linear_q_points", 6144, 192),
                         ("linear_kv_points", 6336, 480)):
        ops.linear_dx((dproj, off, LDP), mv(P[f"{pre}.{name}.weight"]), ds, R, n, CS, beta=True)
        _lin_grads(G, f"{pre}.{name}.weight", f"{pre}.{name}.bias", (dproj, off, LDP), s, R, n, CS)
    return (dzb, sv["W40"]) if defer_dz else None


def ln_skip_fwd(P, b, x1, init_node, R):
    pre = "score_model.trunk"
    dev = x1
    u0 = empty((R, TD), dev)
    mean = empty((R,), dev); rstd = empty((R,), dev)
    ops.layernorm(mv(x1), P[f"{pre}.ipa_ln_{b}.weight"], P[f"{pre}.ipa_ln_{b}.bias"], (u0, 0, TD), R, CS, save=(mean, rstd))
    ops.linear(mv(init_node), mv(P[f"{pre}.skip_embed_{b}.weight"]), P[f"{pre}.skip_embed_{b}.bias"], (u0, CS, TD), R, 64, CS)
    return u0, dict(x1=x1, mean=mean, rstd=rstd, init_node=init_node, R=R)


def ln_skip_bwd(P, G, b, sv, du0, dx1, dinit):
    pre = "score_model.trunk"
    R = sv["R"]
    ops.layernorm_bwd((du0, 0, TD), mv(sv["x1"]), P[f"{pre}.ipa_ln_{b}.weight"], sv["mean"], sv["rstd"], mv(dx1), R, CS,
                      dgamma=G[f"{pre}.ipa_ln_{b}.weight"], dbeta=G[f"{pre}.ipa_ln_{b}.bias"])
    ops.linear_dx((du0, CS, TD), mv(P[f"{pre}.skip_embed_{b}.weight"]), mv(dinit), R, 64, CS, beta=True)
    _lin_grads(G, f"{pre}.skip_embed_{b}.weight", f"{pre}.skip_embed_{b}.bias", (du0, CS, TD), mv(sv["init_node"]), R, 64, CS)


def tfmr_layer_fwd(P, pre, x, key_add, B, N, save=True, out_rowscale=None, x_ln=None, defer_out_ln=False):
    dev = key_add
    R = B * N
    L = lib()
    qkv = empty((R, 3 * TD), dev)
    if x_ln is not None:
        t_in, g_in, b_in, rs_in, lnc, x = x_ln + (0, None)[len(x_ln) - 4:]
        x = empty((R, TD), dev) if x is None else x
        ops.ln_linear(t_in if isinstance(t_in, tuple) else mv(t_in), g_in, b_in, mv(P[f"{pre}.self_attn.in_proj_weight"]), P[f"{pre}.self_attn.in_proj_bias"], mv(qkv),
                      R, 3 * TD, TD, ln_rowscale=rs_in, ln_out=mv(x), ln_cols=lnc)
    else:
        ops.linear(mv(x), mv(P[f"{pre}.self_attn.in_proj_weight"]), P[f"{pre}.self_attn.in_proj_bias"], mv(qkv), R, 3 * TD, TD)
    o = empty((R, TD), dev)
    if opts.fused_seq_attn and R >= opts.seq_attn_min_rows:
        A = empty((B, TH, N, N), dev) if save else None
        L.call("fd_seq_attn_fwd", qkv, key_add, o, A, 1.0 / math.sqrt(THD), B, N)
    else:
        A = empty((B, TH, N, N), dev)
        L.gemm(qkv, qkv, A, N, N, THD, (3 * TD, 1), (1, 3 * TD), N, b_off=TD, batch=B * TH, bdiv=TH,
               a_bs=(N * 3 * TD, THD), b_bs=(N * 3 * TD, THD), c_bs=(TH * N * N, N * N), alpha=1.0 / math.sqrt(THD))
        L.call("fd_row_softmax_fwd", A, key_add, B * TH * N, N, TH * N)
        L.gemm(A, qkv, o, N, THD, N, (N, 1), (3 * TD, 1), TD, b_off=2 * TD, batch=B * TH, bdiv=TH,
               a_bs=(TH * N * N, N * N), b_bs=(N * 3 * TD, THD), c_bs=(N * TD, THD))
    t1 = empty((R, TD), dev)
    ops.linear(mv(o), mv(P[f"{pre}.self_attn.out_proj.weight"]), P[f"{pre}.self_attn.out_proj.bias"], mv(t1), R, TD, TD, resid=mv(x))
    fold = (not save) and ops.ln_linear_ok(mv(t1), mv(P[f"{pre}.linear1.weight"]), R, TD, TD)
    y1 = empty((R, TD), dev); m1 = r1 = None
    f = empty((R, TD), dev)
    if fold:
        ops.ln_linear(mv(t1), P[f"{pre}.norm1.weight"], P[f"{pre}.norm1.bias"], mv(P[f"{pre}.linear1.weight"]),
                      P[f"{pre}.linear1.bias"], mv(f), R, TD, TD, relu=True, ln_out=mv(y1))
# ... 44 lines not shown
        L.call("fd_row_softmax_bwd", A, dA, B * TH * N, N)
        L.gemm(dA, qkv, dqkv, N, THD, N, (N, 1), (3 * TD, 1), 3 * TD, b_off=TD, batch=B * TH, bdiv=TH,
               a_bs=(TH * N * N, N * N), b_bs=(N * 3 * TD, THD), c_bs=(N * 3 * TD, THD), alpha=sc)
        L.gemm(dA, qkv, dqkv, N, THD, N, (1, N), (3 * TD, 1), 3 * TD, c_off=TD, batch=B * TH, bdiv=TH,
               a_bs=(TH * N * N, N * N), b_bs=(N * 3 * TD, THD), c_bs=(N * 3 * TD, THD), alpha=sc)
    _lin_grads(G, f"{pre}.self_attn.in_proj_weight", f"{pre}.self_attn.in_proj_bias", mv(dqkv), mv(sv["x"]), R, 3 * TD, TD)
    dx = empty((R, TD), dev)
    ops.linear_dx(mv(dqkv), mv(P[f"{pre}.self_attn.in_proj_weight"]), mv(dx), R, 3 * TD, TD, resid=mv(dt1))
    return dx


def post_node_fwd(P, b, u2, u0, mask, R, u2_ln=None, defer_ln=False):
    pre = "score_model.trunk"
    dev = u0
    n2 = empty((R, CS), dev)
    if u2_ln is not None:
        t_in, g_in, b_in, rs_in = u2_ln
        ops.ln_linear(mv(t_in), g_in, b_in, mv(P[f"{pre}.post_tfmr_{b}.weight"]), P[f"{pre}.post_tfmr_{b}.bias"], mv(n2), R, CS, TD,
                      resid=(u0, 0, TD), ln_rowscale=rs_in)
    else:
        ops.linear(mv(u2), mv(P[f"{pre}.post_tfmr_{b}.weight"]), P[f"{pre}.post_tfmr_{b}.bias"], mv(n2), R, CS, TD, resid=(u0, 0, TD))
    nt = f"{pre}.node_transition_{b}"
    h1 = empty((R, CS), dev); h2 = empty((R, CS), dev); t = empty((R, CS), dev); n3 = empty((R, CS), dev)
    mean = empty((R,), dev); rstd = empty((R,), dev)
    ops.linear(mv(n2), mv(P[f"{nt}.linear_1.weight"]), P[f"{nt}.linear_1.bias"], mv(h1), R, CS, CS, relu=True)
    ops.linear(mv(h1), mv(P[f"{nt}.linear_2.weight"]), P[f"{nt}.linear_2.bias"], mv(h2), R, CS, CS, relu=True)
    ops.linear(mv(h2), mv(P[f"{nt}.linear_3.weight"]), P[f"{nt}.linear_3.bias"], mv(t), R, CS, CS, resid=mv(n2))
    if defer_ln:
        return None, (t, P[f"{nt}.ln.weight"], P[f"{nt}.ln.bias"], mask, 0, n3)
    ops.layernorm(mv(t), P[f"{nt}.ln.weight"], P[f"{nt}.ln.bias"], mv(n3), R, CS, rowscale=mask, save=(mean, rstd))
    return n3, dict(u2=u2, n2=n2, h1=h1, h2=h2, t=t, mean=mean, rstd=rstd, mask=mask, R=R)


def post_node_bwd(P, G, b, sv, dn3, du0):
    pre = "score_model.trunk"
    nt = f"{pre}.node_transition_{b}"
    R = sv["R"]
    dev = dn3
    dt = empty((R, CS), dev)
    ops.layernorm_bwd(mv(dn3), mv(sv["t"]), P[f"{nt}.ln.weight"], sv["mean"], sv["rstd"], mv(dt), R, CS,
                      rowscale=sv["mask"], dgamma=G[f"{nt}.ln.weight"], dbeta=G[f"{nt}.ln.bias"])
    _lin_grads(G, f"{nt}.linear_3.weight", f"{nt}.linear_3.bias", mv(dt), mv(sv["h2"]), R, CS, CS)
    dh2 = empty((R, CS), dev)
    ops.linear_dx(mv(dt), mv(P[f"{nt}.linear_3.weight"]), mv(dh2), R, CS, CS, gate=mv(sv["h2"]))
    _lin_grads(G, f"{nt}.linear_2.weight", f"{nt}.linear_2.bias", mv(dh2), mv(sv["h1"]), R, CS, CS)
    dh1 = empty((R, CS), dev)
    ops.linear_dx(mv(dh2), mv(P[f"{nt}.linear_2.weight"]), mv(dh1), R, CS, CS, gate=mv(sv["h1"]))
    _lin_grads(G, f"{nt}.linear_1.weight", f"{nt}.linear_1.bias", mv(dh1), mv(sv["n2"]), R, CS, CS)
    dn2 = empty((R, CS), dev)
    ops.linear_dx(mv(dh1), mv(P[f"{nt}.linear_1.weight"]), mv(dn2), R, CS, CS, resid=mv(dt))
    _lin_grads(G, f"{pre}.post_tfmr_{b}.weight", f"{pre}.post_tfmr_{b}.bias", mv(dn2), mv(sv["u2"]), R, CS, TD)
    du2 = empty((R, TD), dev)
    ops.linear_dx(mv(dn2), mv(P[f"{pre}.post_tfmr_{b}.weight"]), mv(du2), R, CS, TD)
    ops.add_view((du0, 0, TD), mv(dn2), R, CS)
    return du2
```

### se3_diffusion_amd/ops.py

```python
from __future__ import annotations

import math
import threading

import torch

from . import hip
from .options import opts

F32 = torch.float32


def lib():
    return hip.get_lib()


def empty(shape, like, dtype=F32):
    return torch.empty(shape, device=like.device, dtype=dtype)


def zeros(shape, like, dtype=F32):
    a = _ARENA["buf"]
    if a is not None and dtype == F32 and a.device == like.device:
        n = 1
# ... 231 lines not shown
    if not q["items"]:
        return
    items, tens, rows = q["items"], q["tensors"], q["rows"]
    q["items"], q["tensors"], q["rows"] = [], [], None
    side(lambda: group_dw(items, rows, blocks), tens, rows)


def add_view(dst, src, rows, cols, alpha=1.0):
    dt, do, dl = dst
    st, so, sl = src
    lib().call("fd_add2d", (dt, do), dl, (st, so), sl, rows, cols, alpha)


def bias_grad(dy, db, M, N):
    dt, do, dl = dy
    lib().call("fd_colsum_acc", (dt, do), dl, M, N, db)


def layernorm(x, gamma, beta, y, rows, C, *, rowscale=None, save=None):
    xt, xo, xl = x
    yt, yo, yl = y
    mean, rstd = save if save is not None else (None, None)
    lib().call("fd_layernorm_fwd", (xt, xo), xl, gamma, beta, rowscale, (yt, yo), yl, mean, rstd, rows, C, 1e-5)


def layernorm_bwd(dy, x, gamma, mean, rstd, dx, rows, C, *, rowscale=None, dgamma=None, dbeta=None, accum=False):
    dt, do, dl = dy
    xt, xo, xl = x
    gt, go, gl = dx
    lib().call("fd_layernorm_bwd", (dt, do), dl, (xt, xo), xl, gamma, rowscale, mean, rstd, (gt, go), gl,
               int(accum), dgamma, dbeta, rows, C)


def ln_linear_ok(x, W, M, N, K):
    return bool(opts.ln_fold and M <= 1024 and K % 8 == 0 and K <= 320 and x[1] % 4 == 0 and W[1] == 0 and x[2] % 4 == 0
                and W[2] % 4 == 0)


def ln_linear(x, gamma, beta, W, b, out, M, N, K, *, relu=False, resid=None, ln_rowscale=None, ln_out=None, ln_cols=0):
    d = hip.FdLnGemmDesc()
    tens = hip.fill_ptrs(d, x=x, gamma=gamma, beta=beta, ln_rowscale=ln_rowscale, ln_out=ln_out, W=W, bias=b, resid=resid, out=out)
    d.ldx, d.ldw, d.ldo = x[2], W[2], out[2]
    if ln_out is not None:
        d.ld_ln_out = ln_out[2]
    if resid is not None:
        d.ld_resid = resid[2]
    d.M, d.N, d.K, d.relu, d.eps, d.ln_cols = int(M), int(N), int(K), int(bool(relu)), 1e-5, int(ln_cols)
    lib().launch("fd_ln_gemm", d, tens)


_TABLES = {}


def feature_tables(device, index_embed_size=32, num_bins=22, min_bin=1e-5, max_bin=20.0):
    key = (str(device), index_embed_size, num_bins, min_bin, max_bin)
    if key not in _TABLES:
        half = index_embed_size // 2
        tfreq = torch.exp(torch.arange(half, dtype=torch.float32) * -(math.log(10000) / (half - 1)))
        k = torch.arange(half)
        idenom = (2056 ** (2 * k[None] / index_embed_size))[0].to(torch.float32)
        lower = torch.linspace(min_bin, max_bin, num_bins)
        upper = torch.cat([lower[1:], lower.new_tensor([1e8])])
        _TABLES[key] = tuple(t.contiguous().to(device) for t in (tfreq, idenom, lower, upper))
    return _TABLES[key]


def edge_mlp_pack(W1, W2, Wf, backward=False, out=None, W40=None):
    img = out if out is not None else torch.empty(hip.EDGE_MLP_IMAGE_BYTES, dtype=torch.uint8, device=W1.device)
    assert W40 is None or (W40.is_contiguous() and tuple(W40.shape) == (40, 128))
    assert W1.stride(-1) == 1 and W2.stride(-1) == 1 and Wf.stride(-1) == 1 and W1.stride(0) == W2.stride(0) == Wf.stride(0)
    ld = W1.stride(0)
    if not backward:
        lib().call("fd_edge_mlp_pack", W1, W2, Wf, ld, img)
        if W40 is not None:
            lib().call("fd_edge_mlp_pack_zb", W40, img)
    else:
        lib().call("fd_edge_mlp_pack_bwd", Wf, W2, W1, ld, W40, img)
    return img


def edge_mlp_pack_bwd(Wf, W2, W1, W40=None, out=None):
    return edge_mlp_pack(W1, W2, Wf, backward=True, out=out, W40=W40)


_SCHED = {}
_SCHED_LOCK = threading.Lock()
STATS = {"edge_dynamic_launches": 0, "ipa_flash_fwd": 0, "ipa_sequence_fwd": 0, "ipa_flash_bwd": 0, "ipa_sequence_bwd": 0,
         "ipa_flash_bwd_keys": 0, "ipa_keys_gemms": 0}


_SCHED_WORDS = 256


def edge_sched_init(device):
    with _SCHED_LOCK:
        pool = _SCHED.get(("pool", device))
        if pool is None:
            if device.type == "cuda" and torch.cuda.is_current_stream_capturing():
                raise RuntimeError("ops.edge_sched_init must run before hipGraph capture starts (sampler.sample calls it)")
            pool = _SCHED[("pool", device)] = (torch.zeros(_SCHED_WORDS, dtype=torch.int32, device=device), {})
    return pool


def _edge_sched(like, stream):
    buf, slots = edge_sched_init(like.device)
    with _SCHED_LOCK:
        key = int(stream or 0)
        slot = slots.get(key)
        if slot is None:
            if len(slots) >= _SCHED_WORDS // 4:
                raise RuntimeError(f"ops._edge_sched: more than {_SCHED_WORDS // 4} streams have used the dynamic tile hand-out on "
                                   f"{like.device}; raise ops._SCHED_WORDS")
            slot = slots[key] = len(slots)
        STATS["edge_dynamic_launches"] += 1
    return buf.data_ptr() + 16 * slot
# ... 84 lines not shown
```

### se3_diffusion_amd/optim.py

```python
from __future__ import annotations

import contextlib

import torch
import torch.distributed as dist

from . import hip

_ALIGN = 64


class FlatAdam:
    def __init__(self, params, lr=1e-4, betas=(0.9, 0.999), eps=1e-8, adjacent=None, max_grad_norm=None,
                 skip_nonfinite=False, ema_decay=None, ema_warmup=True):
        self.params = [p for p in params if p.requires_grad]
        assert self.params, "no trainable parameters"
        assert all(p.dtype == torch.float32 for p in self.params), "fp32 parameters only"
        self.lr, self.betas, self.eps = float(lr), (float(betas[0]), float(betas[1])), float(eps)
        dev = self.params[0].device
        group_of = {}
        for grp in (adjacent or ()):
            grp = [p for p in grp if p.requires_grad]
            assert all(p.numel() % 4 == 0 for p in grp[:-1]), "grouped parameters must keep their successors 16-byte aligned"
            for p in grp:
                group_of[id(p)] = grp
        placed, off = {}, 0
        for p in self.params:
            if id(p) in placed:
                continue
            for q in group_of.get(id(p), [p]):
                if id(q) in placed:
                    continue
                placed[id(q)] = off
                off += q.numel()
            off = (off + _ALIGN - 1) // _ALIGN * _ALIGN
        self.offsets = [placed[id(p)] for p in self.params]
        self.numel = off
        self.flat_p = torch.zeros(off, device=dev)
        self.flat_g = torch.zeros(off, device=dev)
        self.exp_avg = torch.zeros(off, device=dev)
        self.exp_avg_sq = torch.zeros(off, device=dev)
        for p, o in zip(self.params, self.offsets):
            view = self.flat_p[o:o + p.numel()].view_as(p)
            view.copy_(p.data)
            p.data = view
            p.grad = self.flat_g[o:o + p.numel()].view_as(p)
        self.max_grad_norm = None if max_grad_norm is None else float(max_grad_norm)
        self.skip_nonfinite = bool(skip_nonfinite)
        self.guarded = self.max_grad_norm is not None or self.skip_nonfinite
        self._max_norm_arg()
        self._t = 0
        self._ws = self._opt_state = self._stats = None
        if self.guarded:
            self._ws = torch.empty(hip.OPT_WS_DOUBLES, dtype=torch.float64, device=dev)
            self._opt_state = torch.zeros(hip.OPT_STATE_BYTES // 8, dtype=torch.int64, device=dev)
        self._dirty = False
        self.ema_decay = None if ema_decay is None else float(ema_decay)
        self.ema_warmup = bool(ema_warmup)
        self.ema = None
        self._ema_live = False
        if self.ema_decay is not None:
            self._ema_decay_arg()
            self.ema = self.flat_p.clone()

    @property
    def t(self):
        if self.guarded:
            raise AttributeError("a guarded FlatAdam counts its steps on the device: applied_steps() / set_applied_steps()")
        return self._t

    @t.setter
    def t(self, value):
        if self.guarded:
            raise AttributeError("a guarded FlatAdam counts its steps on the device: applied_steps() / set_applied_steps()")
        self._t = int(value)

    def _max_norm_arg(self):
        if self.max_grad_norm is None:
            return 0.0
# ... 197 lines not shown
```

### se3_diffusion_amd/trunk.py

```python
from __future__ import annotations

import math

import numpy as np
import torch

from . import hip, ops
from .trace import rng
from . import network as nw
from .network import CS, CZ, TD, H, _lin_grads
from .ops import empty, zeros, mv, lib
from .options import opts

EH = 384
CE = 128


def bb_update_fwd(P, b, n3, dmask, quat, trans, R):
    pre = f"score_model.trunk.bb_update_{b}.linear"
    dev = n3
    upd = empty((R, 6), dev); q2 = empty((R, 4), dev); t2 = empty((R, 3), dev)
    lib().call("fd_bb_update_fwd", n3, CS, CS, dmask, P[f"{pre}.weight"], P[f"{pre}.bias"], quat, trans, upd, q2, t2, R)
    return q2, t2, dict(n3=n3, dmask=dmask, quat=quat, upd=upd, R=R)


def bb_update_bwd(P, G, b, sv, dq2, dt2, dframe, dn3):
    pre = f"score_model.trunk.bb_update_{b}.linear"
    R = sv["R"]
    dev = dq2
    dq = empty((R, 4), dev); dt = empty((R, 3), dev); dupd = empty((R, 6), dev); dupd_s = empty((R, 6), dev)
    lib().call("fd_bb_update_bwd", dq2, dt2, dframe, sv["dmask"], sv["upd"], sv["quat"], dq, dt, dupd, dupd_s, R)
    if G is not None:
        def _grads():
            ops.linear_dw(mv(dupd_s), mv(sv["n3"]), mv(G[f"{pre}.weight"]), R, 6, CS)
            ops.bias_grad(mv(dupd), G[f"{pre}.bias"], R, 6)
        ops.side(_grads, (dupd_s, dupd, sv["n3"]), R)
    ops.linear_dx(mv(dupd_s), mv(P[f"{pre}.weight"]), mv(dn3), R, 6, CS, beta=True)
    return dq, dt


def _edge_mlp_image(P, pre, cache, backward=False, W40=None):
    key = ("et_img", pre, backward, W40 is not None)
    if cache is not None and key in cache:
        return cache[key]
    img = ops.edge_mlp_pack(P[f"{pre}.trunk.0.weight"], P[f"{pre}.trunk.2.weight"], P[f"{pre}.final_layer.weight"],
                            backward=backward, W40=W40)
    if cache is not None:
        cache[key] = img
    return img


def fused_edge():
    return opts.fused_edge and not lib().exact_f32


def et_folds_node_terms(cache, save):
    return cache is not None and not save and opts.fold_node_terms and fused_edge()


def edge_transition_fwd(P, b, n3, z, emask, B, N, save=True, cache=None, zb_next=None):
    if not fused_edge():
        return edge_transition_fwd_unfused(P, b, n3, z, emask, B, N) + (None,)
    terms = edge_transition_terms(P, b, n3, B * N, save=save, cache=cache)
    return edge_transition_pair(P, b, terms, n3, z, emask, B, N, save=save, cache=cache, zb_next=zb_next)


def edge_transition_terms(P, b, n3, R, save=True, cache=None, n3_ln=None):
    pre = f"score_model.trunk.edge_transition_{b}"
    W1, Wf = P[f"{pre}.trunk.0.weight"], P[f"{pre}.final_layer.weight"]
    assert n3_ln is None or et_folds_node_terms(cache, save)
    if et_folds_node_terms(cache, save):
        LDT = 2 * EH + 2 * CZ
        key = ("et_fold", pre)
        if key not in cache:
            Wi, bi = P[f"{pre}.initial_embed.weight"], P[f"{pre}.initial_embed.bias"]
            Wcat = torch.cat([W1[:, CZ:CZ + CE], W1[:, CZ + CE:], Wf[:, CZ:CZ + CE], Wf[:, CZ + CE:]], 0).contiguous()
            Wfold = empty((LDT, CS), Wi)
# ... 103 lines not shown
    gW1, gWf = G[f"{pre}.trunk.0.weight"], G[f"{pre}.final_layer.weight"]
    z, e, h1, h2 = sv["z"], sv["e"], sv["h1"], sv["h2"]
    fused = sv.get("mh1") is not None and (fused_edge() or bool(sv.get("h2_has_z")))
    h2_has_z = bool(sv.get("h2_has_z"))
    assert fused or not h2_has_z, "a fused edge-transition forward needs the fused backward (its h2 save carries z)"
    fused_ln = fused and opts.fused_ln_bwd and (dzb_next is None or dzb_next[1].is_contiguous())
    grouped_dw = fused and opts.grouped_pair_dw
    dy = empty((Pn, CZ), dev)
    de = empty((R, CE), dev)

    def ln_bwd(dz2):
        if dzb_next is not None:
            acc = dz2 is not None
            dz2 = dz2 if acc else empty((Pn, CZ), dev)
            L.call("fd_ipa_dz_acc", dzb_next[0], dzb_next[1].contiguous(), dz2, Pn, int(acc))
        if flush_behind_launch:
            ops.flush_dw()
        ops.layernorm_bwd(mv(dz2), mv(sv["y"]), P[f"{pre}.layer_norm.weight"], sv["mean"], sv["rstd"], mv(dy), Pn, CZ,
                          rowscale=sv["emask"], dgamma=G[f"{pre}.layer_norm.weight"], dbeta=G[f"{pre}.layer_norm.bias"])

    def final_layer_grads():
        if not grouped_dw:
            def _grads_y():
                ops.linear_dw(mv(dy), mv(h2), mv(gWf), Pn, CZ, EH)
                if not h2_has_z:
                    ops.linear_dw(mv(dy), mv(z), (gWf, 0, EH), Pn, CZ, CZ)
            ops.side(_grads_y, (dy, h2, z), Pn)
        _node_terms_bwd(G, dy, CZ, Wf, gWf, f"{pre}.final_layer.bias", e, de, B, N, accumulate=False)

    if fused:
        dh2 = empty((Pn, EH), dev); dh1 = empty((Pn, EH), dev)
        dx_args = dict(save1=dh2, save2=dh1, backward=True, gmask1=sv["mh2"], gmask2=sv["mh1"])
    if fused_ln:
        img = ops.edge_mlp_pack_bwd(Wf, W2, W1, W40=dzb_next[1] if dzb_next is not None else None)
        ops.edge_mlp(dz2, img, dz, Pn, N, ln_y=sv["y"], ln_mean=sv["mean"], ln_rstd=sv["rstd"],
                     ln_gamma=P[f"{pre}.layer_norm.weight"], ln_rowscale=sv["emask"], dy_out=dy,
                     ln_dgamma=G[f"{pre}.layer_norm.weight"], ln_dbeta=G[f"{pre}.layer_norm.bias"],
                     dzb=dzb_next[0] if dzb_next is not None else None, **dx_args)
        if flush_behind_launch:
            ops.flush_dw()
        final_layer_grads()
    elif fused:
        ln_bwd(dz2)
        final_layer_grads()
        ops.edge_mlp(dy, _edge_mlp_image(P, pre, None, backward=True), dz, Pn, N, **dx_args)
    else:
        ln_bwd(dz2)
        final_layer_grads()
        ops.linear_dx(mv(dy), (Wf, 0, EH), mv(dz), Pn, CZ, CZ)
        dh2 = empty((Pn, EH), dev)
        ops.linear_dx(mv(dy), mv(Wf), mv(dh2), Pn, CZ, EH, gate=mv(h2))
        _lin_grads(G, f"{pre}.trunk.2.weight", f"{pre}.trunk.2.bias", mv(dh2), mv(h1), Pn, EH, EH)
        dh1 = empty((Pn, EH), dev)
        ops.linear_dx(mv(dh2), mv(W2), mv(dh1), Pn, EH, EH, gate=mv(h1))
    if grouped_dw:
        gW2, gb2 = G[f"{pre}.trunk.2.weight"], G[f"{pre}.trunk.2.bias"]
        items = [dict(A=(dh2, 0, EH), B=(h1, CZ * j, EH), C=(gW2, CZ * j, EH), colsum=gb2 if j == 0 else None)
                 for j in range(3)]
        items.append(dict(A=(dh1, 0, EH), B=(z, 0, CZ), C=(gW1, 0, EH)))
        it = dict(A=(h2, 0, EH), B=(dy, 0, CZ), C=(gWf, 0, EH), trans=True)
        if not h2_has_z:
            it["A_add"] = (z, 0, CZ)
        items.append(it)
        nblk = opts.pair_dw_blocks if ops.side_active(dh2, Pn) else 0
        ops.side(lambda: ops.pair_dw(items, Pn, blocks=nblk), (dh2, dh1, h1, h2, z, dy), Pn)
    else:
        if fused:
# ... 69 lines not shown
    R = B * N
    h1 = empty((R, CS), dev); h2 = empty((R, CS), dev); u = empty((R, 2), dev)
    ops.linear(mv(node), mv(P[f"{tp}.linear_1.weight"]), P[f"{tp}.linear_1.bias"], mv(h1), R, CS, CS, relu=True)
    ops.linear(mv(h1), mv(P[f"{tp}.linear_2.weight"]), P[f"{tp}.linear_2.bias"], mv(h2), R, CS, CS, resid=mv(node))
    ops.linear(mv(h2), mv(P[f"{tp}.linear_final.weight"]), P[f"{tp}.linear_final.bias"], mv(u), R, 2, CS)
    hc, sg = head_tables(dconf, dev.device)
    rot = empty((B, N, 3), dev, torch.float64); ts = empty((B, N, 3), dev); rig = empty((B, N, 7), dev)
    psi = empty((B, N, 2), dev); a37 = empty((B, N, 37, 3), dev); a14 = empty((B, N, 14, 3), dev)
    gt = feats["torsion_angles_sin_cos"]
    tt = feats["t"].float().contiguous()
    lib().call("fd_heads_fwd", feats["rigids_t"], quat, trans, u, (gt, 4), 14, feats["fixed_mask"], feats["res_mask"],
               tt, sg, sg.numel(), hc, rot, ts, rig, psi, a37, a14, sc_ca_out, B, N)
    out = dict(psi=psi, rot_score=rot, trans_score=ts, rigids=rig, atom37=a37, atom14=a14)
    return out, dict(node=node, h1=h1, h2=h2, u=u, quat=quat, trans=trans, psi=psi, t=tt, hc=hc, sg=sg, B=B, N=N)


def heads_bwd(P, G, sv, feats, d_out, dnode):
    tp = "score_model.torsion_pred"
    B, N = sv["B"], sv["N"]
    R = B * N
    dev = sv["node"]
    dq = empty((R, 4), dev); dt = empty((R, 3), dev); du = empty((R, 2), dev)

    def g(k, dtype=torch.float32):
        v = d_out.get(k)
        return None if v is None else v.to(dtype).contiguous()

    lib().call("fd_heads_bwd", feats["rigids_t"], sv["quat"], sv["trans"], sv["u"], sv["psi"], feats["fixed_mask"],
               feats["res_mask"], sv["t"], sv["sg"], sv["sg"].numel(), sv["hc"], g("rot_score", torch.float64),
               g("trans_score"), g("rigids"), g("psi"), g("atom37"), dq, dt, du, B, N)
    _lin_grads(G, f"{tp}.linear_final.weight", f"{tp}.linear_final.bias", mv(du), mv(sv["h2"]), R, 2, CS)
    dh2 = empty((R, CS), dev)
    ops.linear_dx(mv(du), mv(P[f"{tp}.linear_final.weight"]), mv(dh2), R, 2, CS)
    ops.add_view(mv(dnode), mv(dh2), R, CS)
    _lin_grads(G, f"{tp}.linear_2.weight", f"{tp}.linear_2.bias", mv(dh2), mv(sv["h1"]), R, CS, CS)
    dh1 = empty((R, CS), dev)
    ops.linear_dx(mv(dh2), mv(P[f"{tp}.linear_2.weight"]), mv(dh1), R, CS, CS, gate=mv(sv["h1"]))
    _lin_grads(G, f"{tp}.linear_1.weight", f"{tp}.linear_1.bias", mv(dh1), mv(sv["node"]), R, CS, CS)
    ops.linear_dx(mv(dh1), mv(P[f"{tp}.linear_1.weight"]), mv(dnode), R, CS, CS, beta=True)
    return dq, dt


def _prep_feats(feats):
    f = {}
    f["res_mask"] = feats["res_mask"].to(torch.float32).contiguous()
    f["fixed_mask"] = feats["fixed_mask"].to(torch.float32).contiguous()
    f["seq_idx"] = feats["seq_idx"].to(torch.int64).contiguous()
    f["t"] = feats["t"].contiguous()
    f["sc_ca_t"] = feats["sc_ca_t"].to(torch.float32).contiguous()
    f["rigids_t"] = feats["rigids_t"].to(torch.float32).contiguous()
    f["torsion_angles_sin_cos"] = feats["torsion_angles_sin_cos"].to(torch.float32).contiguous()
    return f


def _cached(cache, key, fn):
    if cache is None:
        return fn()
    if key not in cache:
        cache[key] = fn()
    return cache[key]


def _tfmr_layers(P, b):
    n = 0
    while f"score_model.trunk.seq_tfmr_{b}.layers.{n}.linear1.weight" in P:
        n += 1
    return n


def forward(P, feats, num_blocks, dconf=(0.1, 0.1, 20.0, 0.1, 1.5, 1000), tfmr_bool_mask=False, save=True, cache=None,
            sc_ca_out=None):
    if save:
        cache = None
    planes = ops.weight_planes(P) if save else None
    if not save:
        ops.set_weight_planes(None)
    f = _prep_feats(feats)
    B, N = f["res_mask"].shape
    R = B * N
    L = lib()
    mask = f["res_mask"]
    dev = mask
    if not (mask.is_cuda and torch.cuda.is_current_stream_capturing()):
        ops.edge_sched_init(mask.device)
    if cache is not None:
        sig = (B, N, mask.data_ptr(), f["fixed_mask"].data_ptr(), bool(tfmr_bool_mask))
        if cache.get("_sig") != sig:
            cache.clear()
            cache["_sig"] = sig
    rig = f["rigids_t"]
    quat = empty((R, 4), dev); trans = empty((R, 3), dev)
    t32 = f["t"].dtype == torch.float32
    tsc = empty((B,), dev) if t32 else None
    L.call("fd_split_rigids", rig, float(dconf[0]), f["t"] if t32 else None, 10000.0, quat, trans, tsc, R, B)
    f["tscaled"] = tsc if t32 else (f["t"] * 10000).float().contiguous()
    with rng("embed.fwd"):
        node0, z, sv_embed, zb = nw.embed_fwd(P, f, B, N, cache, save=save,
                                              zb_next=nw.ipa_w40(P, "score_model.trunk.ipa_0", cache) if num_blocks > 0 else None)
    emask = sv_embed["emask"]

    def _dmask():
        dm = empty((B, N), dev)
        L.call("fd_rowscale", (1 - f["fixed_mask"]).contiguous(), 1, mask.reshape(-1), dm, 1, R, 1)
        return dm
    dmask = _cached(cache, "dmask", _dmask)
    init_node = node0
    node = node0
# ... 48 lines not shown
                                                   x_ln=pend_ln, defer_out_ln=not save)
                sv_t.append(s_)
        with rng(f"node_transition_{b}.fwd"):
            n3, sv_pn = nw.post_node_fwd(P, b, u, u0, mask.view(-1), R, u2_ln=pend_ln, defer_ln=fold6)
            pend_ln = None
        sv_et = None
        if fold6:
            n3_ln, sv_pn = sv_pn, None
            n3 = n3_ln[5]
            with rng(f"edge_transition_{b}.fwd"):
                terms = edge_transition_terms(P, b, None, R, save=save, cache=cache, n3_ln=n3_ln)
                with rng(f"node_transition_{b}.fwd"):
                    q2, t2, sv_bb = bb_update_fwd(P, b, n3, dmask.view(-1), quat, trans, R)
                z, sv_et, zb = edge_transition_pair(P, b, terms, n3, z, emask, B, N, save=save, cache=cache,
                                                    zb_next=nw.ipa_w40(P, f"score_model.trunk.ipa_{b + 1}", cache))
        else:
            with rng(f"node_transition_{b}.fwd"):
                q2, t2, sv_bb = bb_update_fwd(P, b, n3, dmask.view(-1), quat, trans, R)
            if b < num_blocks - 1:
                with rng(f"edge_transition_{b}.fwd"):
                    z, sv_et, zb = edge_transition_fwd(P, b, n3, z, emask, B, N, save=save, cache=cache,
                                                       zb_next=nw.ipa_w40(P, f"score_model.trunk.ipa_{b + 1}", cache))
        stages.append(dict(ipa=sv_ipa, ln=sv_ln, tfmr=sv_t, pn=sv_pn, bb=sv_bb, et=sv_et))
        node, quat, trans = n3, q2, t2
        if not save:
            stages[-1] = None
    with rng("heads.fwd"):
        sc_out = sc_ca_out if not save else None
        assert sc_out is None or (sc_out.is_contiguous() and sc_out.dtype == torch.float32 and tuple(sc_out.shape) == (B, N, 3))
        out, sv_h = heads_fwd(P, node, quat, trans, f, B, N, dconf, sc_ca_out=sc_out)
    if not save:
        return out, None
    return out, dict(feats=f, embed=sv_embed, stages=stages, heads=sv_h, B=B, N=N, num_blocks=num_blocks,
                     bool_mask=tfmr_bool_mask, mask=mask, dmask=dmask, planes=planes)


def backward(P, G, sv, d_out, on_done=None):
    notify = on_done if on_done is not None else (lambda tag: None)
    hooked = on_done is not None
    B, N, nb = sv["B"], sv["N"], sv["num_blocks"]
    R, Pn = B * N, B * N * N
    f = sv["feats"]
    dev = sv["mask"]
    if sv["bool_mask"]:
        raise NotImplementedError("backward is defined for the training-mode (additive) transformer mask")
    ops.reset_dw_queue()
    ops.set_weight_planes(sv.get("planes"))
    try:
        with ops.zero_arena(R * (nb * 2048 + 1024) + 65536 if opts.zero_arena else 0, dev):
            _backward(P, G, sv, d_out, notify, hooked)
    except BaseException:
        ops.reset_dw_queue()
        raise
    finally:
        ops.set_weight_planes(None)


def _backward(P, G, sv, d_out, notify, hooked=False):
    B, N, nb = sv["B"], sv["N"], sv["num_blocks"]
    R, Pn = B * N, B * N * N
    f = sv["feats"]
    dev = sv["mask"]
    dnode = zeros((R, CS), dev)
    nw.embed_regen_early(sv["embed"], G)
    with rng("heads.bwd"):
        dq, dt = heads_bwd(P, G, sv["heads"], f, d_out, dnode)
    ops.flush_dw()
    notify("heads")
    dinit = zeros((R, CS), dev)
    dz = None
    defer_dw = bool(opts.defer_node_dw and not hooked)
    pend = None
    for b in reversed(range(nb)):
        st = sv["stages"][b]
        dn3 = dnode
        dz_in = None
        if st["et"] is not None:
            dz_in = empty((Pn, CZ), dev)
            with rng(f"edge_transition_{b}.bwd"):
                edge_transition_bwd(P, G, b, st["et"], dz, dz_in, dn3, dzb_next=pend, flush_behind_launch=defer_dw)
            pend = None
        dframe = zeros((R, 12), dev)
        with rng(f"node_transition_{b}.bwd"):
            dq_in, dt_in = bb_update_bwd(P, G, b, st["bb"], dq, dt, None, dn3)
            du0 = zeros((R, TD), dev)
            du2 = nw.post_node_bwd(P, G, b, st["pn"], dn3, du0)
        with rng(f"seq_tfmr_{b}.bwd"):
            du = du2
            for l in reversed(range(len(st["tfmr"]))):
                du = nw.tfmr_layer_bwd(P, G, f"score_model.trunk.seq_tfmr_{b}.layers.{l}", st["tfmr"][l], du)
            ops.add_view(mv(du0), mv(du), R, TD)
            dx1 = empty((R, CS), dev)
            nw.ln_skip_bwd(P, G, b, st["ln"], du0, dx1, dinit)
        ds = zeros((R, CS), dev)
        defer = b > 0 and fused_edge() and opts.fused_ln_bwd and sv["stages"][b - 1]["et"] is not None
        dz_acc = dz_in is not None
        if dz_in is None and not defer:
            dz_in = empty((Pn, CZ), dev)
        with rng(f"ipa_{b}.bwd"):
            pend = nw.ipa_bwd(P, G, f"score_model.trunk.ipa_{b}", st["ipa"], dx1, mv(ds), dz_in, dframe, dz_accumulate=dz_acc,
                              defer_dz=defer)
        _frame_grad_fold(st["bb"]["quat"], dframe, dq_in, dt_in, R)
        dq, dt, dnode, dz = dq_in, dt_in, ds, dz_in
        if not (defer_dw and b > 0 and sv["stages"][b - 1]["et"] is not None):
            ops.flush_dw()
        notify(b)
    ops.add_view(mv(dnode), mv(dinit), R, CS)
    with rng("embed.bwd"):
        nw.embed_bwd(P, G, sv["embed"], dnode, dz)
    ops.flush_dw()
    notify("embed")
    ops.join_grad_stream()


def _frame_grad_fold(quat, dframe, dq, dt, R):
    dev = quat
    z4 = zeros((R, 4), dev); z3 = zeros((R, 3), dev); z6 = zeros((R, 6), dev); zm = zeros((R,), dev)
    dq2 = empty((R, 4), dev); dt2 = empty((R, 3), dev); j1 = empty((R, 6), dev); j2 = empty((R, 6), dev)
    lib().call("fd_bb_update_bwd", z4, z3, dframe, zm, z6, quat, dq2, dt2, j1, j2, R)
    ops.add_view(mv(dq), mv(dq2), R, 4)
    ops.add_view(mv(dt), mv(dt2), R, 3)
```

Before: 182,000.

## Batch weight-image packing per step and fuse backward glue kernels

Packs all edge-transition and edge-embedder weight images once per step in a single multi-item launch and reuses them in forward and backward. The frame-gradient fold becomes one dedicated kernel instead of zero-filled buffers, a full bb_update_bwd call and two adds. Residual adds and zero-fills in the node-transition and layer-norm skip backward are folded into a two-input layernorm backward and a resid argument on linear_dx. The tile-counter memset is replaced by a self-resetting atomic. Together these target launch count and small elementwise traffic, at the cost of more complex shared state between forward and backward and new correctness risks in the counter reset.

```diff
diff --git a/include/fd_hip.h b/include/fd_hip.h
--- a/include/fd_hip.h
+++ b/include/fd_hip.h
@@ -55,6 +55,10 @@
 int fd_layernorm_bwd(const float* dy, long lddy, const float* x, long ldx, const float* gamma,
                      const float* rowscale, const float* mean, const float* rstd, float* dx, long lddx,
                      int dx_accum, float* dgamma, float* dbeta, long rows, int C, void* stream);
+int fd_layernorm_bwd2(const float* dy, long lddy, const float* dy2, long lddy2, const float* x, long ldx, const float* gamma,
+                      const float* rowscale, const float* mean, const float* rstd, float* dx, long lddx, int dx_accum,
+                      const float* rowscale2, float* dx_scaled, long ld_scaled, float* dgamma, float* dbeta, long rows, int C,
+                      void* stream);
 int fd_colsum_acc(const float* X, long ld, long rows, int ncols, float* out, void* stream);
 int fd_pair_reduce_acc(const float* X, int nbatch, int n, int C, float* rowsum, float* colsum, long ld_out,
                        void* stream);
@@ -66,6 +70,21 @@
 int fd_edge_mlp_pack_zb(const float* W40, void* image, void* stream);
 int fd_edge_mlp_pack(const float* W1, const float* W2, const float* Wf, long ld, void* image, void* stream);
 int fd_edge_mlp_pack_bwd(const float* Wf, const float* W2, const float* W1, long ld, const float* W40, void* image, void* stream);
+#define FD_PACK_EDGE_FWD 0
+#define FD_PACK_EDGE_BWD 1
+#define FD_PACK_EMBED_FWD 2
+#define FD_PACK_EMBED_BWD 3
+#define FD_PACK_MAX_ITEMS 16
+typedef struct FdPackItem {
+  const float* w0;
+  const float* w1;
+  const float* w2;
+  const float* W40;
+  void* image;
+  long ld;
+  int kind;
+} FdPackItem;
+int fd_pack_images(const FdPackItem* items, int n, void* stream);
 typedef struct FdEdgeMlpDesc {
   const float* x;
   const void* img;
@@ -305,6 +324,7 @@
 int fd_bb_update_bwd(const float* dquat_out, const float* dtrans_out, const float* dframe, const float* dmask,
                      const float* upd, const float* quat, float* dquat, float* dtrans, float* dupd, float* dupd_s,
                      long R, void* stream);
+int fd_frame_grad_fold(const float* quat, const float* dframe, float* dquat, float* dtrans, long R, void* stream);
 
 typedef struct FdHeadConst {
   float atoms[15];
diff --git a/se3_diffusion_amd/csrc/fd_edge_embed.hip b/se3_diffusion_amd/csrc/fd_edge_embed.hip
--- a/se3_diffusion_amd/csrc/fd_edge_embed.hip
+++ b/se3_diffusion_amd/csrc/fd_edge_embed.hip
@@ -11,52 +11,20 @@
 constexpr int EE_C = 128;
 constexpr float kPi = 3.14159265358979323846f;
 
+#include "fd_pack_image.h"
+static_assert(PK_EE_UNITS == EE_UNITS && PK_ZB_UNITS == EE_ZB_UNITS && PK_ZB == EE_ZB && PK_C == EE_C, "fd_pack_image.h: edge-embedder image");
+
 __global__ __launch_bounds__(256) void edge_embed_pack_kernel(const float* __restrict__ W0, const float* __restrict__ W2,
                                                               const float* __restrict__ W4, char* __restrict__ img) {
   const int gid = (int)(blockIdx.x * blockDim.x + threadIdx.x);
   if (gid >= EE_UNITS * 4 * 64) return;
-  const int lane = gid & 63, i = (gid >> 6) & 3, u = gid >> 8;
-  const int m = lane & 15, g = lane >> 4;
-  const int layer = u < 4 ? 0 : (u < 12 ? 1 : 2);
-  const int r = u - (layer == 0 ? 0 : (layer == 1 ? 4 : 12));
-  const int n = 64 * (r & 1) + 16 * i + m, k0 = 32 * (r >> 1);
-  float x[8];
-#pragma unroll
-  for (int e = 0; e < 8; ++e) {
-    if (layer == 0) {
-      const int k = k0 + 8 * g + e;
-      x[e] = k < 54 ? W0[n * 120 + 66 + k] : 0.f;
-    } else {
-      const int k = k0 + 16 * (e >> 2) + 4 * g + (e & 3);
-      x[e] = (layer == 1 ? W2 : W4)[n * EE_C + k];
-    }
-  }
-  uint4 s0, s1, s2;
-  em_split8(x, s0, s1, s2);
-  char* dst = img + (long)u * EM_UNIT + (i * 3) * EM_PIECE + lane * 16;
-  *reinterpret_cast<uint4*>(dst) = s0;
-  *reinterpret_cast<uint4*>(dst + EM_PIECE) = s1;
-  *reinterpret_cast<uint4*>(dst + 2 * EM_PIECE) = s2;
+  pk_embed(W0, W2, W4, img, gid >> 8, (gid >> 6) & 3, gid & 63);
 }
 
 __global__ __launch_bounds__(256) void edge_embed_pack_zb_kernel(const float* __restrict__ W40, char* __restrict__ img) {
   const int gid = (int)(blockIdx.x * blockDim.x + threadIdx.x);
   if (gid >= EE_ZB_UNITS * 4 * 64) return;
-  const int lane = gid & 63, i = (gid >> 6) & 3, ks = gid >> 8;
-  const int m = lane & 15, g = lane >> 4;
-  const int n = 16 * i + m;
-  float x[8];
-#pragma unroll
-  for (int e = 0; e < 8; ++e) {
-    const int k = 32 * ks + 16 * (e >> 2) + 4 * g + (e & 3);
-    x[e] = n < EE_ZB ? W40[n * EE_C + k] : 0.f;
-  }
-  uint4 s0, s1, s2;
-  em_split8(x, s0, s1, s2);
-  char* dst = img + (long)(EE_UNITS + ks) * EM_UNIT + (i * 3) * EM_PIECE + lane * 16;
-  *reinterpret_cast<uint4*>(dst) = s0;
-  *reinterpret_cast<uint4*>(dst + EM_PIECE) = s1;
-  *reinterpret_cast<uint4*>(dst + 2 * EM_PIECE) = s2;
+  pk_zb(W40, img + (long)EE_UNITS * EM_UNIT, gid >> 8, (gid >> 6) & 3, gid & 63);
 }
 
 template <bool ZB>
diff --git a/se3_diffusion_amd/csrc/fd_edge_embed_bwd.hip b/se3_diffusion_amd/csrc/fd_edge_embed_bwd.hip
--- a/se3_diffusion_amd/csrc/fd_edge_embed_bwd.hip
+++ b/se3_diffusion_amd/csrc/fd_edge_embed_bwd.hip
@@ -8,28 +8,15 @@
 constexpr int EB_UNITS = 16;
 constexpr int EB_NSTAGE = EB_UNITS / EM_UPS;
 constexpr int EB_C = 128;
+
+#include "fd_pack_image.h"
+static_assert(PK_EB_UNITS == EB_UNITS && PK_C == EB_C, "fd_pack_image.h: edge-embedder backward image");
 
 __global__ __launch_bounds__(256) void edge_embed_bwd_pack_kernel(const float* __restrict__ W2, const float* __restrict__ W4,
                                                                   char* __restrict__ img) {
   const int gid = (int)(blockIdx.x * blockDim.x + threadIdx.x);
   if (gid >= EB_UNITS * 4 * 64) return;
-  const int lane = gid & 63, i = (gid >> 6) & 3, u = gid >> 8;
-  const int m = lane & 15, g = lane >> 4;
-  const int layer = u >> 3, r = u & 7;
-  const int n = 64 * (r & 1) + 16 * i + m, k0 = 32 * (r >> 1);
-  const float* __restrict__ W = layer == 0 ? W4 : W2;
-  float x[8];
-#pragma unroll
-  for (int e = 0; e < 8; ++e) {
-    const int k = k0 + 16 * (e >> 2) + 4 * g + (e & 3);
-    x[e] = W[k * EB_C + n];
-  }
-  uint4 s0, s1, s2;
-  em_split8(x, s0, s1, s2);
-  char* dst = img + (long)u * EM_UNIT + (i * 3) * EM_PIECE + lane * 16;
-  *reinterpret_cast<uint4*>(dst) = s0;
-  *reinterpret_cast<uint4*>(dst + EM_PIECE) = s1;
-  *reinterpret_cast<uint4*>(dst + 2 * EM_PIECE) = s2;
+  pk_embed_bwd(W2, W4, img, gid >> 8, (gid >> 6) & 3, gid & 63);
 }
 
 __global__ __launch_bounds__(64 * EM_WAVES, 2) void edge_embed_bwd_kernel(FdEdgeEmbedBwdDesc d) {
@@ -77,7 +64,11 @@
 
   int tile = first, nxt = 0;
   for (int ti = 0;;) {
-    if (dyn && tid == 0) nxt = G + (int)atomicAdd(&sched[0], 1u);
+    if (dyn && tid == 0) {
+      const unsigned got = atomicAdd(&sched[0], 1u);
+      if (got == (unsigned)(ntiles - 1)) atomicAdd(&sched[0], 0u - (unsigned)ntiles);
+      nxt = G + (int)got;
+    }
     const long row = (long)tile * EM_ROWS + wave * 16 + m;
     const bool rok = row < rows;
     const long rc = rok ? row : rows - 1;
@@ -276,12 +267,7 @@
   const int blocks = d.blocks > 0 ? d.blocks : 256 * EM_BLOCKS_PER_CU;
   const long grid = ntiles < blocks ? ntiles : blocks;
   FdEdgeEmbedBwdDesc dd = d;
-  if (dd.sched != nullptr && ntiles >= 4 * grid) {
-    FD_CHECK_ARG(hipMemsetAsync(dd.sched, 0, sizeof(unsigned), (hipStream_t)stream) == hipSuccess,
-                 "fd_edge_embed_bwd: zeroing the tile counter failed");
-  } else {
-    dd.sched = nullptr;
-  }
+  if (!(dd.sched != nullptr && ntiles >= 4 * grid)) dd.sched = nullptr;
   hipLaunchKernelGGL(edge_embed_bwd_kernel, dim3((unsigned)grid), dim3(64 * EM_WAVES), 0, (hipStream_t)stream, dd);
   FD_CHECK_LAUNCH("fd_edge_embed_bwd");
   return FD_OK;
diff --git a/se3_diffusion_amd/csrc/fd_edge_mlp.hip b/se3_diffusion_amd/csrc/fd_edge_mlp.hip
--- a/se3_diffusion_amd/csrc/fd_edge_mlp.hip
+++ b/se3_diffusion_amd/csrc/fd_edge_mlp.hip
@@ -47,82 +47,70 @@
 #endif
 
 #ifndef EM_SHAPE_W8
-struct EmMat {
-  const float* p;
-  long rs, cs;
-};
+#include "fd_pack_image.h"
+static_assert(PK_EM_UNITS == EM_UNITS && PK_ZB_UNITS == EM_ZB_UNITS && PK_ZB == EM_ZB && PK_C == EM_C, "fd_pack_image.h: edge-transition image");
 
 __global__ __launch_bounds__(256) void edge_mlp_pack16_kernel(EmMat A1, EmMat A2, EmMat A4, char* __restrict__ img, int rot) {
   const int gid = (int)(blockIdx.x * blockDim.x + threadIdx.x);
   if (gid >= EM_UNITS * 4 * 64) return;
-  const int lane = gid & 63, i = (gid >> 6) & 3, u = gid >> 8;
-  const int m = lane & 15, g = lane >> 4;
-  EmMat M;
-  int n, k0;
-  if (u < 96) {
-    const int c = u / 32, r = u % 32, hc = (c + rot) % 3;
-    if (r < 8) {
-      M = A1; n = 128 * hc + 64 * (r & 1) + 16 * i + m; k0 = 32 * (r >> 1);
-    } else {
-      const int r2 = r - 8;
-      M = A2; n = 64 * (r2 % 6) + 16 * i + m; k0 = 128 * hc + 32 * (r2 / 6);
-    }
-  } else {
-    const int v = u - 96;
-    M = A4; n = 64 * (v & 1) + 16 * i + m; k0 = 32 * (v >> 1);
-  }
-  float x[8];
-#pragma unroll
-  for (int e = 0; e < 8; ++e) {
-    const int k = k0 + 16 * (e >> 2) + 4 * g + (e & 3);
-    x[e] = M.p[(long)n * M.rs + (long)k * M.cs];
-  }
-  uint4 s0, s1, s2;
-  em_split8(x, s0, s1, s2);
-  char* dst = img + (long)u * EM_UNIT + (i * 3) * EM_PIECE + lane * 16;
-  *reinterpret_cast<uint4*>(dst) = s0;
-  *reinterpret_cast<uint4*>(dst + EM_PIECE) = s1;
-  *reinterpret_cast<uint4*>(dst + 2 * EM_PIECE) = s2;
+  pk_edge16(A1, A2, A4, img, rot, gid >> 8, (gid >> 6) & 3, gid & 63);
 }
 
 __global__ __launch_bounds__(256) void edge_mlp_pack_zb_kernel(const float* __restrict__ W40, char* __restrict__ img) {
   const int gid = (int)(blockIdx.x * blockDim.x + threadIdx.x);
   if (gid >= EM_ZB_UNITS * 4 * 64) return;
-  const int lane = gid & 63, i = (gid >> 6) & 3, ks = gid >> 8;
-  const int m = lane & 15, g = lane >> 4;
-  const int n = 16 * i + m;
-  float x[8];
-#pragma unroll
-  for (int e = 0; e < 8; ++e) {
-    const int k = 32 * ks + 16 * (e >> 2) + 4 * g + (e & 3);
-    x[e] = n < EM_ZB ? W40[n * EM_C + k] : 0.f;
-  }
-  uint4 s0, s1, s2;
-  em_split8(x, s0, s1, s2);
-  char* dst = img + (long)(EM_UNITS + ks) * EM_UNIT + (i * 3) * EM_PIECE + lane * 16;
-  *reinterpret_cast<uint4*>(dst) = s0;
-  *reinterpret_cast<uint4*>(dst + EM_PIECE) = s1;
-  *reinterpret_cast<uint4*>(dst + 2 * EM_PIECE) = s2;
+  pk_zb(W40, img + (long)EM_UNITS * EM_UNIT, gid >> 8, (gid >> 6) & 3, gid & 63);
 }
 
 __global__ __launch_bounds__(256) void edge_mlp_pack_zbw_kernel(const float* __restrict__ W40, char* __restrict__ img) {
   const int gid = (int)(blockIdx.x * blockDim.x + threadIdx.x);
   if (gid >= EM_ZB_UNITS * 4 * 64) return;
-  const int lane = gid & 63, i = (gid >> 6) & 3, u = gid >> 8;
-  const int m = lane & 15, g = lane >> 4;
-  const int n = 64 * (u & 1) + 16 * i + m, k0 = 32 * (u >> 1);
-  float x[8];
-#pragma unroll
-  for (int e = 0; e < 8; ++e) {
-    const int k = k0 + 8 * g + e;
-    x[e] = k < EM_ZB ? W40[k * EM_C + n] : 0.f;
-  }
-  uint4 s0, s1, s2;
-  em_split8(x, s0, s1, s2);
-  char* dst = img + (long)u * EM_UNIT + (i * 3) * EM_PIECE + lane * 16;
-  *reinterpret_cast<uint4*>(dst) = s0;
-  *reinterpret_cast<uint4*>(dst + EM_PIECE) = s1;
-  *reinterpret_cast<uint4*>(dst + 2 * EM_PIECE) = s2;
+  pk_zbw(W40, img, gid >> 8, (gid >> 6) & 3, gid & 63);
+}
+
+struct PackArgs {
+  FdPackItem item[FD_PACK_MAX_ITEMS];
+  int first[FD_PACK_MAX_ITEMS + 1];
+  int n;
+};
+
+__device__ __host__ inline int pack_item_units(const FdPackItem& it) {
+  const int zb = it.W40 != nullptr ? PK_ZB_UNITS : 0;
+  switch (it.kind) {
+    case FD_PACK_EDGE_FWD: return PK_EM_UNITS + zb;
+    case FD_PACK_EDGE_BWD: return PK_EM_UNITS + zb;
+    case FD_PACK_EMBED_FWD: return PK_EE_UNITS + zb;
+    default: return PK_EB_UNITS;
+  }
+}
+
+__global__ __launch_bounds__(256) void pack_images_kernel(PackArgs a) {
+  const int blk = (int)blockIdx.x;
+  int t = 0;
+  while (t + 1 < a.n && blk >= a.first[t + 1]) ++t;
+  const FdPackItem& it = a.item[t];
+  const int u = blk - a.first[t];
+  const int i = (int)(threadIdx.x >> 6), lane = (int)(threadIdx.x & 63);
+  char* img = static_cast<char*>(it.image);
+  if (it.kind == FD_PACK_EDGE_FWD) {
+    if (u < PK_EM_UNITS)
+      pk_edge16(EmMat{it.w0, it.ld, 1}, EmMat{it.w1, it.ld, 1}, EmMat{it.w2, it.ld, 1}, img, 0, u, i, lane);
+    else
+      pk_zb(it.W40, img + (long)PK_EM_UNITS * EM_UNIT, u - PK_EM_UNITS, i, lane);
+  } else if (it.kind == FD_PACK_EDGE_BWD) {
+    const int lead = it.W40 != nullptr ? PK_ZB_UNITS : 0;
+    if (u < lead)
+      pk_zbw(it.W40, img, u, i, lane);
+    else
+      pk_edge16(EmMat{it.w2, 1, it.ld}, EmMat{it.w1, 1, it.ld}, EmMat{it.w0, 1, it.ld}, img + (long)lead * EM_UNIT, 1, u - lead, i, lane);
+  } else if (it.kind == FD_PACK_EMBED_FWD) {
+    if (u < PK_EE_UNITS)
+      pk_embed(it.w0, it.w1, it.w2, img, u, i, lane);
+    else
+      pk_zb(it.W40, img + (long)PK_EE_UNITS * EM_UNIT, u - PK_EE_UNITS, i, lane);
+  } else {
+    pk_embed_bwd(it.w0, it.w1, img, u, i, lane);
+  }
 }
 
 #endif
@@ -199,7 +187,11 @@
 
   int tile = first, nxt = 0;
   for (int ti = 0;;) {
-    if (dyn && tid == 0) nxt = G + (int)atomicAdd(&sched[0], 1u);
+    if (dyn && tid == 0) {
+      const unsigned got = atomicAdd(&sched[0], 1u);
+      if (got == (unsigned)(ntiles - 1)) atomicAdd(&sched[0], 0u - (unsigned)ntiles);
+      nxt = G + (int)got;
+    }
     const long row = (long)tile * EM_ROWS + wave * 16 + m;
     const bool rok = row < rows;
     const long rc = rok ? row : rows - 1;
@@ -609,11 +601,7 @@
   const int grid = (int)(ntiles < blocks ? ntiles : blocks);
   const dim3 g3(grid), b3(64 * EM_WAVES);
   FdEdgeMlpDesc dd = d;
-  if (dd.sched != nullptr && ntiles >= 4L * grid) {
-    FD_CHECK_ARG(hipMemsetAsync(dd.sched, 0, sizeof(unsigned), st) == hipSuccess, "fd_edge_mlp: zeroing the tile counter failed");
-  } else {
-    dd.sched = nullptr;
-  }
+  if (!(dd.sched != nullptr && ntiles >= 4L * grid)) dd.sched = nullptr;
   const bool zbv = d.zb_out != nullptr, train = d.save1 != nullptr;
 #define EM_GO(...) hipLaunchKernelGGL(HIP_KERNEL_NAME(edge_mlp16_kernel<__VA_ARGS__>), g3, b3, 0, st, dd)
   if (d.backward) {
@@ -662,6 +650,28 @@
   hipLaunchKernelGGL(edge_mlp_pack_zb_kernel, dim3(EM_ZB_UNITS * 4 * 64 / 256), dim3(256), 0, (hipStream_t)stream, W40,
                      static_cast<char*>(img));
   FD_CHECK_LAUNCH("fd_edge_mlp_pack_zb");
+  return FD_OK;
+}
+
+extern "C" int fd_pack_images(const FdPackItem* items, int n, void* stream) {
+  FD_CHECK_ARG(n >= 0 && n <= FD_PACK_MAX_ITEMS && (n == 0 || items != nullptr), "fd_pack_images: 0..%d items", FD_PACK_MAX_ITEMS);
+  if (n == 0) return FD_OK;
+  PackArgs a;
+  a.n = n;
+  int blocks = 0;
+  for (int t = 0; t < n; ++t) {
+    const FdPackItem& it = items[t];
+    FD_CHECK_ARG(it.kind >= FD_PACK_EDGE_FWD && it.kind <= FD_PACK_EMBED_BWD, "fd_pack_images: item %d: unknown kind", t);
+    FD_CHECK_ARG(it.w0 && it.w1 && (it.w2 || it.kind == FD_PACK_EMBED_BWD) && it.image, "fd_pack_images: item %d: null operand", t);
+    FD_CHECK_ARG(fd_aligned16(it.image), "fd_pack_images: item %d: image must be 16-byte aligned", t);
+    FD_CHECK_ARG(it.W40 == nullptr || it.kind != FD_PACK_EMBED_BWD, "fd_pack_images: item %d: the embedder backward image has no W40", t);
+    a.item[t] = it;
+    a.first[t] = blocks;
+    blocks += pack_item_units(it);
+  }
+  for (int t = n; t <= FD_PACK_MAX_ITEMS; ++t) a.first[t] = blocks;
+  hipLaunchKernelGGL(pack_images_kernel, dim3(blocks), dim3(256), 0, (hipStream_t)stream, a);
+  FD_CHECK_LAUNCH("fd_pack_images");
   return FD_OK;
 }
 
diff --git a/se3_diffusion_amd/csrc/fd_frames.hip b/se3_diffusion_amd/csrc/fd_frames.hip
--- a/se3_diffusion_amd/csrc/fd_frames.hip
+++ b/se3_diffusion_amd/csrc/fd_frames.hip
@@ -164,6 +164,22 @@
     dtrans[r * 3 + 0] = dt0; dtrans[r * 3 + 1] = dt1; dtrans[r * 3 + 2] = dt2;
 #pragma unroll
     for (int k = 0; k < 6; ++k) { dupd[r * 6 + k] = du[k]; dupd_s[r * 6 + k] = du[k] * d; }
+  }
+}
+
+__global__ __launch_bounds__(256) void frame_grad_fold_kernel(const float* __restrict__ quat, const float* __restrict__ dframe,
+                                                              float* __restrict__ dquat, float* __restrict__ dtrans, long R_) {
+  for (long r = (long)blockIdx.x * 256 + threadIdx.x; r < R_; r += (long)gridDim.x * 256) {
+    const float* f = dframe + r * 12;
+    float G[9];
+#pragma unroll
+    for (int k = 0; k < 9; ++k) G[k] = f[k];
+    float dq[4] = {0.f, 0.f, 0.f, 0.f};
+    rot_grad_to_quat(quat + r * 4, G, dq);
+#pragma unroll
+    for (int k = 0; k < 4; ++k) dquat[r * 4 + k] += dq[k];
+#pragma unroll
+    for (int k = 0; k < 3; ++k) dtrans[r * 3 + k] += f[9 + k];
   }
 }
 
@@ -580,6 +596,16 @@
   return FD_OK;
 }
 
+extern "C" int fd_frame_grad_fold(const float* quat, const float* dframe, float* dquat, float* dtrans, long R_, void* stream) {
+  FD_CHECK_ARG(R_ >= 0 && (R_ == 0 || (quat && dframe && dquat && dtrans)), "fd_frame_grad_fold: null operand");
+  if (R_ == 0) return FD_OK;
+  long g = (R_ + 255) / 256;
+  hipLaunchKernelGGL(frame_grad_fold_kernel, dim3((unsigned)(g > 4096 ? 4096 : g)), dim3(256), 0, (hipStream_t)stream, quat, dframe,
+                     dquat, dtrans, R_);
+  FD_CHECK_LAUNCH("fd_frame_grad_fold");
+  return FD_OK;
+}
+
 static HeadConst make_hc(const FdHeadConst* c) {
   HeadConst hc;
   for (int i = 0; i < 15; ++i) hc.atoms[i] = c->atoms[i];
diff --git a/se3_diffusion_amd/csrc/fd_norm.hip b/se3_diffusion_amd/csrc/fd_norm.hip
--- a/se3_diffusion_amd/csrc/fd_norm.hip
+++ b/se3_diffusion_amd/csrc/fd_norm.hip
@@ -99,12 +99,19 @@
 }
 
 constexpr int LNB_U = 4;
-template <int NCH>
+struct LnBwdExt {
+  const float* dy2;
+  long lddy2;
+  const float* rowscale2;
+  float* dx2;
+  long lddx2;
+};
+template <int NCH, bool EXT = false>
 __global__ __launch_bounds__(256) void layernorm_bwd4_kernel(
     const float* __restrict__ dy, long lddy, const float* __restrict__ x, long ldx,
     const float* __restrict__ gamma, const float* __restrict__ rowscale, const float* __restrict__ mean,
     const float* __restrict__ rstd, float* __restrict__ dx, long lddx, int dx_accum,
-    float* __restrict__ dgamma, float* __restrict__ dbeta, long rows, int C) {
+    float* __restrict__ dgamma, float* __restrict__ dbeta, long rows, int C, LnBwdExt ext) {
   __shared__ float red[2][4][512];
   const int lane = fd::lane_id(), wave = fd::wave_id();
   int col[NCH];
@@ -123,7 +130,7 @@
   const long wslot = (long)blockIdx.x * 4 + wave, nwaves = (long)gridDim.x * 4;
   for (long base = wslot * LNB_U; base < rows; base += nwaves * LNB_U) {
     float4 xv[LNB_U][NCH], dv[LNB_U][NCH], old[LNB_U][NCH];
-    float m[LNB_U], rr[LNB_U], rs[LNB_U];
+    float m[LNB_U], rr[LNB_U], rs[LNB_U], rs2[LNB_U];
 #pragma unroll
     for (int u = 0; u < LNB_U; ++u) {
       const long r = base + u < rows ? base + u : rows - 1;
@@ -131,11 +138,16 @@
       for (int k = 0; k < NCH; ++k) {
         xv[u][k] = *reinterpret_cast<const float4*>(x + r * ldx + col[k]);
         dv[u][k] = *reinterpret_cast<const float4*>(dy + r * lddy + col[k]);
+        if (EXT && ext.dy2 != nullptr) {
+          const float4 d2 = *reinterpret_cast<const float4*>(ext.dy2 + r * ext.lddy2 + col[k]);
+          dv[u][k] = make_float4(dv[u][k].x + d2.x, dv[u][k].y + d2.y, dv[u][k].z + d2.z, dv[u][k].w + d2.w);
+        }
         if (dx_accum) old[u][k] = *reinterpret_cast<const float4*>(dx + r * lddx + col[k]);
       }
       m[u] = mean[r];
       rr[u] = rstd[r];
       rs[u] = rowscale ? rowscale[r] : 1.f;
+      if (EXT) rs2[u] = (ext.dx2 != nullptr && ext.rowscale2 != nullptr) ? ext.rowscale2[r] : 1.f;
     }
     float4 xh[LNB_U][NCH], g[LNB_U][NCH];
     float s1[LNB_U], s2[LNB_U];
@@ -175,6 +187,9 @@
         o.w = rr[u] * (g[u][k].w - s1[u] - xh[u][k].w * s2[u]);
         if (dx_accum) { o.x += old[u][k].x; o.y += old[u][k].y; o.z += old[u][k].z; o.w += old[u][k].w; }
         *reinterpret_cast<float4*>(dx + (base + u) * lddx + col[k]) = o;
+        if (EXT && ext.dx2 != nullptr)
+          *reinterpret_cast<float4*>(ext.dx2 + (base + u) * ext.lddx2 + col[k]) =
+              make_float4(o.x * rs2[u], o.y * rs2[u], o.z * rs2[u], o.w * rs2[u]);
       }
     }
   }
@@ -536,17 +551,41 @@
   int grid = (int)(g < 1 ? 1 : (g > 1024 ? 1024 : g));
   if (ln128_ok(x, ldx) && ln128_ok(dy, lddy) && ln128_ok(dx, lddx) && fd_aligned16(gamma)) {
     if (C <= 256)
-      hipLaunchKernelGGL(layernorm_bwd4_kernel<1>, dim3(grid), dim3(256), 0, (hipStream_t)stream, dy, lddy, x, ldx, gamma,
-                         rowscale, mean, rstd, dx, lddx, dx_accum, dgamma, dbeta, rows, C);
+      hipLaunchKernelGGL(HIP_KERNEL_NAME(layernorm_bwd4_kernel<1, false>), dim3(grid), dim3(256), 0, (hipStream_t)stream, dy, lddy, x,
+                         ldx, gamma, rowscale, mean, rstd, dx, lddx, dx_accum, dgamma, dbeta, rows, C, LnBwdExt{});
     else
-      hipLaunchKernelGGL(layernorm_bwd4_kernel<2>, dim3(grid), dim3(256), 0, (hipStream_t)stream, dy, lddy, x, ldx, gamma,
-                         rowscale, mean, rstd, dx, lddx, dx_accum, dgamma, dbeta, rows, C);
+      hipLaunchKernelGGL(HIP_KERNEL_NAME(layernorm_bwd4_kernel<2, false>), dim3(grid), dim3(256), 0, (hipStream_t)stream, dy, lddy, x,
+                         ldx, gamma, rowscale, mean, rstd, dx, lddx, dx_accum, dgamma, dbeta, rows, C, LnBwdExt{});
     FD_CHECK_LAUNCH("fd_layernorm_bwd(x4)");
     return FD_OK;
   }
   hipLaunchKernelGGL(layernorm_bwd_kernel, dim3(grid), dim3(256), 0, (hipStream_t)stream, dy, lddy, x, ldx, gamma,
                      rowscale, mean, rstd, dx, lddx, dx_accum, dgamma, dbeta, rows, C);
   FD_CHECK_LAUNCH("fd_layernorm_bwd");
+  return FD_OK;
+}
+
+extern "C" int fd_layernorm_bwd2(const float* dy, long lddy, const float* dy2, long lddy2, const float* x, long ldx,
+                                 const float* gamma, const float* rowscale, const float* mean, const float* rstd, float* dx,
+                                 long lddx, int dx_accum, const float* rowscale2, float* dx_scaled, long ld_scaled,
+                                 float* dgamma, float* dbeta, long rows, int C, void* stream) {
+  FD_CHECK_ARG(C % 64 == 0 && C <= 64 * MAXC_PER_LANE, "fd_layernorm_bwd2: C=%d must be a multiple of 64 <= 512", C);
+  FD_CHECK_ARG((dgamma == nullptr) == (dbeta == nullptr), "fd_layernorm_bwd2: dgamma/dbeta come together");
+  FD_CHECK_ARG(dy && x && gamma && mean && rstd && dx, "fd_layernorm_bwd2: null operand");
+  FD_CHECK_ARG(ln128_ok(x, ldx) && ln128_ok(dy, lddy) && ln128_ok(dx, lddx) && fd_aligned16(gamma) &&
+                   (dy2 == nullptr || ln128_ok(dy2, lddy2)) && (dx_scaled == nullptr || ln128_ok(dx_scaled, ld_scaled)),
+               "fd_layernorm_bwd2: operands must be 16-byte aligned with row strides that are multiples of 4");
+  if (rows == 0) return FD_OK;
+  long g = (rows + 15) / 16;
+  int grid = (int)(g < 1 ? 1 : (g > 1024 ? 1024 : g));
+  const LnBwdExt ext{dy2, lddy2, rowscale2, dx_scaled, ld_scaled};
+  if (C <= 256)
+    hipLaunchKernelGGL(HIP_KERNEL_NAME(layernorm_bwd4_kernel<1, true>), dim3(grid), dim3(256), 0, (hipStream_t)stream, dy, lddy, x,
+                       ldx, gamma, rowscale, mean, rstd, dx, lddx, dx_accum, dgamma, dbeta, rows, C, ext);
+  else
+    hipLaunchKernelGGL(HIP_KERNEL_NAME(layernorm_bwd4_kernel<2, true>), dim3(grid), dim3(256), 0, (hipStream_t)stream, dy, lddy, x,
+                       ldx, gamma, rowscale, mean, rstd, dx, lddx, dx_accum, dgamma, dbeta, rows, C, ext);
+  FD_CHECK_LAUNCH("fd_layernorm_bwd2");
   return FD_OK;
 }
 
diff --git a/se3_diffusion_amd/csrc/fd_pack_image.h b/se3_diffusion_amd/csrc/fd_pack_image.h
--- /dev/null
+++ b/se3_diffusion_amd/csrc/fd_pack_image.h
@@ -0,0 +1,106 @@
+#pragma once
+
+constexpr int PK_EM_UNITS = 120;
+constexpr int PK_ZB_UNITS = 4;
+constexpr int PK_EE_UNITS = 20;
+constexpr int PK_EB_UNITS = 16;
+constexpr int PK_ZB = 40, PK_C = 128;
+
+struct EmMat {
+  const float* p;
+  long rs, cs;
+};
+
+__device__ __forceinline__ void pk_store(char* __restrict__ unit, int i, int lane, const float (&x)[8]) {
+  uint4 s0, s1, s2;
+  em_split8(x, s0, s1, s2);
+  char* dst = unit + (i * 3) * EM_PIECE + lane * 16;
+  *reinterpret_cast<uint4*>(dst) = s0;
+  *reinterpret_cast<uint4*>(dst + EM_PIECE) = s1;
+  *reinterpret_cast<uint4*>(dst + 2 * EM_PIECE) = s2;
+}
+
+__device__ __forceinline__ void pk_edge16(const EmMat& A1, const EmMat& A2, const EmMat& A4, char* __restrict__ img, int rot, int u,
+                                          int i, int lane) {
+  const int m = lane & 15, g = lane >> 4;
+  EmMat M;
+  int n, k0;
+  if (u < 96) {
+    const int c = u / 32, r = u % 32, hc = (c + rot) % 3;
+    if (r < 8) {
+      M = A1; n = 128 * hc + 64 * (r & 1) + 16 * i + m; k0 = 32 * (r >> 1);
+    } else {
+      const int r2 = r - 8;
+      M = A2; n = 64 * (r2 % 6) + 16 * i + m; k0 = 128 * hc + 32 * (r2 / 6);
+    }
+  } else {
+    const int v = u - 96;
+    M = A4; n = 64 * (v & 1) + 16 * i + m; k0 = 32 * (v >> 1);
+  }
+  float x[8];
+#pragma unroll
+  for (int e = 0; e < 8; ++e) {
+    const int k = k0 + 16 * (e >> 2) + 4 * g + (e & 3);
+    x[e] = M.p[(long)n * M.rs + (long)k * M.cs];
+  }
+  pk_store(img + (long)u * EM_UNIT, i, lane, x);
+}
+
+__device__ __forceinline__ void pk_zb(const float* __restrict__ W40, char* __restrict__ img, int ks, int i, int lane) {
+  const int m = lane & 15, g = lane >> 4;
+  const int n = 16 * i + m;
+  float x[8];
+#pragma unroll
+  for (int e = 0; e < 8; ++e) {
+    const int k = 32 * ks + 16 * (e >> 2) + 4 * g + (e & 3);
+    x[e] = n < PK_ZB ? W40[n * PK_C + k] : 0.f;
+  }
+  pk_store(img + (long)ks * EM_UNIT, i, lane, x);
+}
+
+__device__ __forceinline__ void pk_zbw(const float* __restrict__ W40, char* __restrict__ img, int u, int i, int lane) {
+  const int m = lane & 15, g = lane >> 4;
+  const int n = 64 * (u & 1) + 16 * i + m, k0 = 32 * (u >> 1);
+  float x[8];
+#pragma unroll
+  for (int e = 0; e < 8; ++e) {
+    const int k = k0 + 8 * g + e;
+    x[e] = k < PK_ZB ? W40[k * PK_C + n] : 0.f;
+  }
+  pk_store(img + (long)u * EM_UNIT, i, lane, x);
+}
+
+__device__ __forceinline__ void pk_embed(const float* __restrict__ W0, const float* __restrict__ W2, const float* __restrict__ W4,
+                                         char* __restrict__ img, int u, int i, int lane) {
+  const int m = lane & 15, g = lane >> 4;
+  const int layer = u < 4 ? 0 : (u < 12 ? 1 : 2);
+  const int r = u - (layer == 0 ? 0 : (layer == 1 ? 4 : 12));
+  const int n = 64 * (r & 1) + 16 * i + m, k0 = 32 * (r >> 1);
+  float x[8];
+#pragma unroll
+  for (int e = 0; e < 8; ++e) {
+    if (layer == 0) {
+      const int k = k0 + 8 * g + e;
+      x[e] = k < 54 ? W0[n * 120 + 66 + k] : 0.f;
+    } else {
+      const int k = k0 + 16 * (e >> 2) + 4 * g + (e & 3);
+      x[e] = (layer == 1 ? W2 : W4)[n * PK_C + k];
+    }
+  }
+  pk_store(img + (long)u * EM_UNIT, i, lane, x);
+}
+
+__device__ __forceinline__ void pk_embed_bwd(const float* __restrict__ W2, const float* __restrict__ W4, char* __restrict__ img, int u,
+                                             int i, int lane) {
+  const int m = lane & 15, g = lane >> 4;
+  const int layer = u >> 3, r = u & 7;
+  const int n = 64 * (r & 1) + 16 * i + m, k0 = 32 * (r >> 1);
+  const float* __restrict__ W = layer == 0 ? W4 : W2;
+  float x[8];
+#pragma unroll
+  for (int e = 0; e < 8; ++e) {
+    const int k = k0 + 16 * (e >> 2) + 4 * g + (e & 3);
+    x[e] = W[k * PK_C + n];
+  }
+  pk_store(img + (long)u * EM_UNIT, i, lane, x);
+}
diff --git a/se3_diffusion_amd/hip.py b/se3_diffusion_amd/hip.py
--- a/se3_diffusion_amd/hip.py
+++ b/se3_diffusion_amd/hip.py
@@ -116,6 +116,15 @@
 
 EDGE_EMBED_BWD_IMAGE_BYTES = 16 * 12288
 
+PACK_EDGE_FWD, PACK_EDGE_BWD, PACK_EMBED_FWD, PACK_EMBED_BWD = 0, 1, 2, 3
+PACK_MAX_ITEMS = 16
+
+
+class FdPackItem(Structure):
+    __slots__ = ()
+    _fields_ = [("w0", c_void_p), ("w1", c_void_p), ("w2", c_void_p), ("W40", c_void_p), ("image", c_void_p), ("ld", c_long),
+                ("kind", c_int)]
+
 class FdLnGemmDesc(Structure):
     __slots__ = ()
     _fields_ = [
@@ -204,6 +213,7 @@
     "fd_gemm_set_persistent_blocks": "i",
     "fd_edge_mlp_pack": "ppplps",
     "fd_edge_mlp": "Ss",
+    "fd_pack_images": "Sis",
     "fd_edge_mlp_pack_zb": "pps",
     "fd_edge_mlp_pack_bwd": "ppplpps",
     "fd_edge_embed_pack": "pppps",
@@ -216,6 +226,7 @@
     "fd_group_dw": "Ss",
     "fd_layernorm_fwd": "plpppplpplifs",
     "fd_layernorm_bwd": "plplpppppl" + "ipplis",
+    "fd_layernorm_bwd2": "plplplpppppl" + "ippl" + "pplis",
     "fd_colsum_acc": "pllips",
     "fd_pair_reduce_acc": "piiippls",
     "fd_axpby": "ppffls",
@@ -248,6 +259,7 @@
     "fd_split_rigids": "pfpfppplis",
     "fd_bb_update_fwd": "plipppppppp" + "ls",
     "fd_bb_update_bwd": "pppppppppp" + "ls",
+    "fd_frame_grad_fold": "ppppls",
     "fd_heads_fwd": "pppp" + "pl" + "ppp" + "pi" + "S" + "ppppppp" + "iis",
     "fd_heads_bwd": "ppppp" + "ppp" + "pi" + "S" + "ppppp" + "ppp" + "iis",
     "fd_backbone_atoms": "ppSppls",
diff --git a/se3_diffusion_amd/network.py b/se3_diffusion_amd/network.py
--- a/se3_diffusion_amd/network.py
+++ b/se3_diffusion_amd/network.py
@@ -58,12 +58,16 @@
     return y, dict(x=x, h1=h1, h2=h2, h3=h3, mean=mean, rstd=rstd, rowscale=rowscale, M=M, K0=K0, C=Cc)
 
 
-def mlp3_ln_bwd(P, G, pre, sv, dy):
+def mlp3_ln_bwd(P, G, pre, sv, dy, dy2=None):
     M, K0, Cc = sv["M"], sv["K0"], sv["C"]
     dev = dy
     dh3 = empty((M, Cc), dev)
-    ops.layernorm_bwd(mv(dy), mv(sv["h3"]), P[f"{pre}.5.weight"], sv["mean"], sv["rstd"], mv(dh3), M, Cc,
-                      rowscale=sv["rowscale"], dgamma=G[f"{pre}.5.weight"], dbeta=G[f"{pre}.5.bias"])
+    if dy2 is not None:
+        ops.layernorm_bwd2(mv(dy), mv(sv["h3"]), P[f"{pre}.5.weight"], sv["mean"], sv["rstd"], mv(dh3), M, Cc, dy2=mv(dy2),
+                           rowscale=sv["rowscale"], dgamma=G[f"{pre}.5.weight"], dbeta=G[f"{pre}.5.bias"])
+    else:
+        ops.layernorm_bwd(mv(dy), mv(sv["h3"]), P[f"{pre}.5.weight"], sv["mean"], sv["rstd"], mv(dh3), M, Cc,
+                          rowscale=sv["rowscale"], dgamma=G[f"{pre}.5.weight"], dbeta=G[f"{pre}.5.bias"])
     _lin_grads(G, f"{pre}.4.weight", f"{pre}.4.bias", mv(dh3), mv(sv["h2"]), M, Cc, Cc)
     dh2 = empty((M, Cc), dev)
     ops.linear_dx(mv(dh3), mv(P[f"{pre}.4.weight"]), mv(dh2), M, Cc, Cc, gate=mv(sv["h2"]))
@@ -126,7 +130,9 @@
     if cache is not None and key in cache:
         img = cache[key]
     else:
-        img = ops.edge_embed_pack(W0, P[f"{pre}.2.weight"], P[f"{pre}.4.weight"], W40=zb_next[0] if use_zb else None)
+        img = ops.step_image("ee_fwd", W0, P[f"{pre}.2.weight"], P[f"{pre}.4.weight"], zb_next[0] if use_zb else None)
+        if img is None:
+            img = ops.edge_embed_pack(W0, P[f"{pre}.2.weight"], P[f"{pre}.4.weight"], W40=zb_next[0] if use_zb else None)
         if cache is not None:
             cache[key] = img
     edge = empty((Pn, CZ), dev)
@@ -166,8 +172,8 @@
     se["x_early"] = ef
 
 
-def embed_bwd(P, G, sv, dnode, dedge):
-    mlp3_ln_bwd(P, G, "embedding_layer.node_embedder", sv["node"], dnode)
+def embed_bwd(P, G, sv, dnode, dedge, dnode2=None):
+    mlp3_ln_bwd(P, G, "embedding_layer.node_embedder", sv["node"], dnode, dy2=dnode2)
     se = sv["edge"]
     if se.get("x_early") is not None:
         se = dict(se, x=mv(se.pop("x_early")))
@@ -182,7 +188,9 @@
             and all(f"{pre}.{l}.{t}" in G for l in (0, 2, 4) for t in ("weight", "bias"))):
         M = se["M"]
         dh3 = empty((M, CZ), dedge); dh2 = empty((M, CZ), dedge); dh1 = empty((M, CZ), dedge)
-        img = ops.edge_embed_bwd_pack(P[f"{pre}.2.weight"], P[f"{pre}.4.weight"])
+        img = ops.step_image("ee_bwd", P[f"{pre}.2.weight"], P[f"{pre}.4.weight"])
+        if img is None:
+            img = ops.edge_embed_bwd_pack(P[f"{pre}.2.weight"], P[f"{pre}.4.weight"])
         ops.edge_embed_bwd(dedge, se["h3"], se["mean"], se["rstd"], P[f"{pre}.5.weight"], se["rowscale"], se["h2"], se["h1"], img,
                            dh3, dh2, dh1, G[f"{pre}.5.weight"], G[f"{pre}.5.bias"], M, gmask2=se.get("mh2"), gmask1=se.get("mh1"))
         x = se["x"]
@@ -316,17 +324,13 @@
     return x1, sv
 
 
-def ipa_bwd(P, G, pre, sv, dx1, ds, dz, dframe, dz_accumulate=True, defer_dz=False):
+def ipa_bwd(P, G, pre, sv, dm, ds, dz, dframe, dz_accumulate=True, defer_dz=False):
     B, N = sv["B"], sv["N"]
     R, Pn = B * N, B * N * N
-    dev = dx1
+    dev = dm
     L = lib()
-    mask = sv["mask"]
     s, z, proj, A, feats, zb = sv["s"], sv["z"], sv["proj"], sv["A"], sv["feats"], sv["zb"]
     quat, qp, kp, vp = sv["quat"], sv["qp"], sv["kp"], sv["vp"]
-    dm = empty((R, CS), dev)
-    L.call("fd_rowscale", dx1, CS, mask, dm, CS, R, CS)
-    ops.add_view(ds, mv(dx1), R, CS)
     _lin_grads(G, f"{pre}.linear_out.weight", f"{pre}.linear_out.bias", mv(dm), mv(feats), R, CS, LDF)
     dfeats = empty((R, LDF), dev)
     ops.linear_dx(mv(dm), mv(P[f"{pre}.linear_out.weight"]), mv(dfeats), R, CS, LDF)
@@ -419,13 +423,14 @@
     return u0, dict(x1=x1, mean=mean, rstd=rstd, init_node=init_node, R=R)
 
 
-def ln_skip_bwd(P, G, b, sv, du0, dx1, dinit):
+def ln_skip_bwd(P, G, b, sv, du, dn2, dx1, dm, mask, dinit):
     pre = "score_model.trunk"
     R = sv["R"]
-    ops.layernorm_bwd((du0, 0, TD), mv(sv["x1"]), P[f"{pre}.ipa_ln_{b}.weight"], sv["mean"], sv["rstd"], mv(dx1), R, CS,
-                      dgamma=G[f"{pre}.ipa_ln_{b}.weight"], dbeta=G[f"{pre}.ipa_ln_{b}.bias"])
-    ops.linear_dx((du0, CS, TD), mv(P[f"{pre}.skip_embed_{b}.weight"]), mv(dinit), R, 64, CS, beta=True)
-    _lin_grads(G, f"{pre}.skip_embed_{b}.weight", f"{pre}.skip_embed_{b}.bias", (du0, CS, TD), mv(sv["init_node"]), R, 64, CS)
+    ops.layernorm_bwd2((du, 0, TD), mv(sv["x1"]), P[f"{pre}.ipa_ln_{b}.weight"], sv["mean"], sv["rstd"], mv(dx1), R, CS,
+                       dy2=mv(dn2), rowscale2=mask, dx_scaled=mv(dm),
+                       dgamma=G[f"{pre}.ipa_ln_{b}.weight"], dbeta=G[f"{pre}.ipa_ln_{b}.bias"])
+    ops.linear_dx((du, CS, TD), mv(P[f"{pre}.skip_embed_{b}.weight"]), mv(dinit), R, 64, CS, beta=True)
+    _lin_grads(G, f"{pre}.skip_embed_{b}.weight", f"{pre}.skip_embed_{b}.bias", (du, CS, TD), mv(sv["init_node"]), R, 64, CS)
 
 
 def tfmr_layer_fwd(P, pre, x, key_add, B, N, save=True, out_rowscale=None, x_ln=None, defer_out_ln=False):
@@ -536,7 +541,7 @@
     return n3, dict(u2=u2, n2=n2, h1=h1, h2=h2, t=t, mean=mean, rstd=rstd, mask=mask, R=R)
 
 
-def post_node_bwd(P, G, b, sv, dn3, du0):
+def post_node_bwd(P, G, b, sv, dn3):
     pre = "score_model.trunk"
     nt = f"{pre}.node_transition_{b}"
     R = sv["R"]
@@ -556,5 +561,4 @@
     _lin_grads(G, f"{pre}.post_tfmr_{b}.weight", f"{pre}.post_tfmr_{b}.bias", mv(dn2), mv(sv["u2"]), R, CS, TD)
     du2 = empty((R, TD), dev)
     ops.linear_dx(mv(dn2), mv(P[f"{pre}.post_tfmr_{b}.weight"]), mv(du2), R, CS, TD)
-    ops.add_view((du0, 0, TD), mv(dn2), R, CS)
-    return du2
+    return du2, dn2
diff --git a/se3_diffusion_amd/ops.py b/se3_diffusion_amd/ops.py
--- a/se3_diffusion_amd/ops.py
+++ b/se3_diffusion_amd/ops.py
@@ -287,6 +287,17 @@
                int(accum), dgamma, dbeta, rows, C)
 
 
+def layernorm_bwd2(dy, x, gamma, mean, rstd, dx, rows, C, *, dy2=None, rowscale=None, rowscale2=None, dx_scaled=None, dgamma=None,
+                   dbeta=None, accum=False):
+    dt, do, dl = dy
+    xt, xo, xl = x
+    gt, go, gl = dx
+    d2 = (dy2[0], dy2[1]) if dy2 is not None else None
+    sc = (dx_scaled[0], dx_scaled[1]) if dx_scaled is not None else None
+    lib().call("fd_layernorm_bwd2", (dt, do), dl, d2, dy2[2] if dy2 is not None else 0, (xt, xo), xl, gamma, rowscale, mean, rstd,
+               (gt, go), gl, int(accum), rowscale2, sc, dx_scaled[2] if dx_scaled is not None else 0, dgamma, dbeta, rows, C)
+
+
 def ln_linear_ok(x, W, M, N, K):
     return bool(opts.ln_fold and M <= 1024 and K % 8 == 0 and K <= 320 and x[1] % 4 == 0 and W[1] == 0 and x[2] % 4 == 0
                 and W[2] % 4 == 0)
@@ -336,6 +347,89 @@
 
 def edge_mlp_pack_bwd(Wf, W2, W1, W40=None, out=None):
     return edge_mlp_pack(W1, W2, Wf, backward=True, out=out, W40=W40)
+
+
+_IMAGES = None
+_PARAM_BUFFERS = []
+
+
+def register_param_buffer(t):
+    import weakref
+    _PARAM_BUFFERS[:] = [r for r in _PARAM_BUFFERS if r() is not None]
+    _PARAM_BUFFERS.append(weakref.ref(t))
+
+
+def _versions(ts):
+    bufs = [b for b in (r() for r in _PARAM_BUFFERS) if b is not None]
+    out = []
+    for t in ts:
+        a, own = t.data_ptr(), -1
+        for b in bufs:
+            if b.device == t.device and b.data_ptr() <= a < b.data_ptr() + b.numel() * b.element_size():
+                own = b._version
+                break
+        out.append((t._version, own))
+    return tuple(out)
+
+
+_PACK_BYTES = {hip.PACK_EDGE_FWD: hip.EDGE_MLP_IMAGE_BYTES, hip.PACK_EDGE_BWD: hip.EDGE_MLP_IMAGE_BYTES,
+               hip.PACK_EMBED_FWD: hip.EDGE_EMBED_IMAGE_BYTES, hip.PACK_EMBED_BWD: hip.EDGE_EMBED_BWD_IMAGE_BYTES}
+
+
+def pack_images(items):
+    for lo in range(0, len(items), hip.PACK_MAX_ITEMS):
+        chunk = items[lo:lo + hip.PACK_MAX_ITEMS]
+        arr = (hip.FdPackItem * len(chunk))()
+        for e, (kind, w0, w1, w2, W40, img) in zip(arr, chunk):
+            ws = [w for w in (w0, w1, w2) if w is not None]
+            assert all(w.stride(-1) == 1 and w.dtype == F32 for w in ws)
+            assert W40 is None or (W40.is_contiguous() and tuple(W40.shape) == (40, 128))
+            assert img.numel() * img.element_size() >= _PACK_BYTES[kind]
+            if kind in (hip.PACK_EDGE_FWD, hip.PACK_EDGE_BWD):
+                assert w0.stride(0) == w1.stride(0) == w2.stride(0)
+                e.ld = w0.stride(0)
+            else:
+                assert all(w.is_contiguous() for w in ws)
+            hip.fill_ptrs(e, w0=w0, w1=w1, w2=w2, W40=W40, image=img)
+            e.kind = int(kind)
+        lib().call("fd_pack_images", arr, len(chunk))
+
+
+def pack_step_images(specs):
+    if not specs:
+        return None
+    dev = specs[0][2].device
+    offs, total = [], 0
+    for sp in specs:
+        offs.append(total)
+        total += _PACK_BYTES[sp[1]]
+    buf = torch.empty(total, dtype=torch.uint8, device=dev)
+    items, imgs = [], {}
+    for (key, kind, w0, w1, w2, W40), o in zip(specs, offs):
+        img = buf[o:o + _PACK_BYTES[kind]]
+        items.append((kind, w0, w1, w2, W40, img))
+        src = tuple(t for t in (w0, w1, w2, W40) if t is not None)
+        imgs[key] = (img, src, _versions(src))
+    pack_images(items)
+    return imgs
+
+
+def set_step_images(imgs):
+    global _IMAGES
+    was, _IMAGES = _IMAGES, imgs
+    return was
+
+
+def step_image(key, *src):
+    ent = _IMAGES.get(key) if _IMAGES is not None else None
+    if ent is None:
+        return None
+    img, was, ver = ent
+    src = tuple(t for t in src if t is not None)
+    if (len(src) != len(was) or any(a.data_ptr() != b.data_ptr() or a.stride() != b.stride() for a, b in zip(src, was))
+            or _versions(src) != ver):
+        return None
+    return img
 
 
 _SCHED = {}
diff --git a/se3_diffusion_amd/optim.py b/se3_diffusion_amd/optim.py
--- a/se3_diffusion_amd/optim.py
+++ b/se3_diffusion_amd/optim.py
@@ -5,7 +5,7 @@
 import torch
 import torch.distributed as dist
 
-from . import hip
+from . import hip, ops
 
 _ALIGN = 64
 
@@ -45,6 +45,7 @@
             view.copy_(p.data)
             p.data = view
             p.grad = self.flat_g[o:o + p.numel()].view_as(p)
+        ops.register_param_buffer(self.flat_p)
         self.max_grad_norm = None if max_grad_norm is None else float(max_grad_norm)
         self.skip_nonfinite = bool(skip_nonfinite)
         self.guarded = self.max_grad_norm is not None or self.skip_nonfinite
diff --git a/se3_diffusion_amd/trunk.py b/se3_diffusion_amd/trunk.py
--- a/se3_diffusion_amd/trunk.py
+++ b/se3_diffusion_amd/trunk.py
@@ -43,6 +43,10 @@
     key = ("et_img", pre, backward, W40 is not None)
     if cache is not None and key in cache:
         return cache[key]
+    img = ops.step_image(("et_bwd" if backward else "et_fwd", pre), P[f"{pre}.trunk.0.weight"], P[f"{pre}.trunk.2.weight"],
+                         P[f"{pre}.final_layer.weight"], W40)
+    if img is not None:
+        return img
     img = ops.edge_mlp_pack(P[f"{pre}.trunk.0.weight"], P[f"{pre}.trunk.2.weight"], P[f"{pre}.final_layer.weight"],
                             backward=backward, W40=W40)
     if cache is not None:
@@ -212,7 +216,7 @@
         dh2 = empty((Pn, EH), dev); dh1 = empty((Pn, EH), dev)
         dx_args = dict(save1=dh2, save2=dh1, backward=True, gmask1=sv["mh2"], gmask2=sv["mh1"])
     if fused_ln:
-        img = ops.edge_mlp_pack_bwd(Wf, W2, W1, W40=dzb_next[1] if dzb_next is not None else None)
+        img = _edge_mlp_image(P, pre, None, backward=True, W40=dzb_next[1] if dzb_next is not None else None)
         ops.edge_mlp(dz2, img, dz, Pn, N, ln_y=sv["y"], ln_mean=sv["mean"], ln_rstd=sv["rstd"],
                      ln_gamma=P[f"{pre}.layer_norm.weight"], ln_rowscale=sv["emask"], dy_out=dy,
                      ln_dgamma=G[f"{pre}.layer_norm.weight"], ln_dbeta=G[f"{pre}.layer_norm.bias"],
@@ -348,12 +352,11 @@
     _lin_grads(G, f"{tp}.linear_final.weight", f"{tp}.linear_final.bias", mv(du), mv(sv["h2"]), R, 2, CS)
     dh2 = empty((R, CS), dev)
     ops.linear_dx(mv(du), mv(P[f"{tp}.linear_final.weight"]), mv(dh2), R, 2, CS)
-    ops.add_view(mv(dnode), mv(dh2), R, CS)
     _lin_grads(G, f"{tp}.linear_2.weight", f"{tp}.linear_2.bias", mv(dh2), mv(sv["h1"]), R, CS, CS)
     dh1 = empty((R, CS), dev)
     ops.linear_dx(mv(dh2), mv(P[f"{tp}.linear_2.weight"]), mv(dh1), R, CS, CS, gate=mv(sv["h1"]))
     _lin_grads(G, f"{tp}.linear_1.weight", f"{tp}.linear_1.bias", mv(dh1), mv(sv["node"]), R, CS, CS)
-    ops.linear_dx(mv(dh1), mv(P[f"{tp}.linear_1.weight"]), mv(dnode), R, CS, CS, beta=True)
+    ops.linear_dx(mv(dh1), mv(P[f"{tp}.linear_1.weight"]), mv(dnode), R, CS, CS, resid=mv(dh2))
     return dq, dt
 
 
@@ -384,11 +387,44 @@
     return n
 
 
+def _pack_step_images(P, num_blocks):
+    specs = []
+    w40 = {}
+
+    def W40(b):
+        if b not in w40:
+            W, bias = nw.ipa_w40(P, f"score_model.trunk.ipa_{b}")
+            w40[b] = W if (W.is_contiguous() and W.data_ptr() % 16 == 0 and bias.data_ptr() % 16 == 0) else None
+        return w40[b]
+
+    if fused_edge():
+        for b in range(num_blocks - 1):
+            pre = f"score_model.trunk.edge_transition_{b}"
+            ws = (P[f"{pre}.trunk.0.weight"], P[f"{pre}.trunk.2.weight"], P[f"{pre}.final_layer.weight"])
+            if not (all(w.stride(-1) == 1 for w in ws) and ws[0].stride(0) == ws[1].stride(0) == ws[2].stride(0)):
+                continue
+            specs.append((("et_fwd", pre), hip.PACK_EDGE_FWD, *ws, W40(b + 1) if opts.zb_from_edge else None))
+            if opts.fused_ln_bwd:
+                specs.append((("et_bwd", pre), hip.PACK_EDGE_BWD, *ws, nw.ipa_w40(P, f"score_model.trunk.ipa_{b + 1}")[0]))
+            else:
+                specs.append((("et_bwd", pre), hip.PACK_EDGE_BWD, *ws, None))
+    if nw.fused_embed():
+        pre = "embedding_layer.edge_embedder"
+        ws = (P[f"{pre}.0.weight"], P[f"{pre}.2.weight"], P[f"{pre}.4.weight"])
+        if all(w.is_contiguous() for w in ws):
+            specs.append(("ee_fwd", hip.PACK_EMBED_FWD, *ws, W40(0) if (opts.zb_from_edge and num_blocks > 0) else None))
+            if opts.fused_embed_bwd:
+                specs.append(("ee_bwd", hip.PACK_EMBED_BWD, ws[1], ws[2], None, None))
+    return ops.pack_step_images(specs)
+
+
 def forward(P, feats, num_blocks, dconf=(0.1, 0.1, 20.0, 0.1, 1.5, 1000), tfmr_bool_mask=False, save=True, cache=None,
             sc_ca_out=None):
     if save:
         cache = None
     planes = ops.weight_planes(P) if save else None
+    images = _pack_step_images(P, num_blocks) if save else None
+    ops.set_step_images(images)
     if not save:
         ops.set_weight_planes(None)
     f = _prep_feats(feats)
@@ -503,7 +539,7 @@
     if not save:
         return out, None
     return out, dict(feats=f, embed=sv_embed, stages=stages, heads=sv_h, B=B, N=N, num_blocks=num_blocks,
-                     bool_mask=tfmr_bool_mask, mask=mask, dmask=dmask, planes=planes)
+                     bool_mask=tfmr_bool_mask, mask=mask, dmask=dmask, planes=planes, images=images)
 
 
 def backward(P, G, sv, d_out, on_done=None):
@@ -517,14 +553,16 @@
         raise NotImplementedError("backward is defined for the training-mode (additive) transformer mask")
     ops.reset_dw_queue()
     ops.set_weight_planes(sv.get("planes"))
+    ops.set_step_images(sv.get("images"))
     try:
-        with ops.zero_arena(R * (nb * 2048 + 1024) + 65536 if opts.zero_arena else 0, dev):
+        with ops.zero_arena(R * (nb * 1088 + 512) + 65536 if opts.zero_arena else 0, dev):
             _backward(P, G, sv, d_out, notify, hooked)
     except BaseException:
         ops.reset_dw_queue()
         raise
     finally:
         ops.set_weight_planes(None)
+        ops.set_step_images(None)
 
 
 def _backward(P, G, sv, d_out, notify, hooked=False):
@@ -532,7 +570,7 @@
     R, Pn = B * N, B * N * N
     f = sv["feats"]
     dev = sv["mask"]
-    dnode = zeros((R, CS), dev)
+    dnode = empty((R, CS), dev)
     nw.embed_regen_early(sv["embed"], G)
     with rng("heads.bwd"):
         dq, dt = heads_bwd(P, G, sv["heads"], f, d_out, dnode)
@@ -554,40 +592,31 @@
         dframe = zeros((R, 12), dev)
         with rng(f"node_transition_{b}.bwd"):
             dq_in, dt_in = bb_update_bwd(P, G, b, st["bb"], dq, dt, None, dn3)
-            du0 = zeros((R, TD), dev)
-            du2 = nw.post_node_bwd(P, G, b, st["pn"], dn3, du0)
+            du2, dn2 = nw.post_node_bwd(P, G, b, st["pn"], dn3)
         with rng(f"seq_tfmr_{b}.bwd"):
             du = du2
             for l in reversed(range(len(st["tfmr"]))):
                 du = nw.tfmr_layer_bwd(P, G, f"score_model.trunk.seq_tfmr_{b}.layers.{l}", st["tfmr"][l], du)
-            ops.add_view(mv(du0), mv(du), R, TD)
-            dx1 = empty((R, CS), dev)
-            nw.ln_skip_bwd(P, G, b, st["ln"], du0, dx1, dinit)
-        ds = zeros((R, CS), dev)
+            ds = empty((R, CS), dev); dm = empty((R, CS), dev)
+            nw.ln_skip_bwd(P, G, b, st["ln"], du, dn2, ds, dm, st["ipa"]["mask"], dinit)
         defer = b > 0 and fused_edge() and opts.fused_ln_bwd and sv["stages"][b - 1]["et"] is not None
         dz_acc = dz_in is not None
         if dz_in is None and not defer:
             dz_in = empty((Pn, CZ), dev)
         with rng(f"ipa_{b}.bwd"):
-            pend = nw.ipa_bwd(P, G, f"score_model.trunk.ipa_{b}", st["ipa"], dx1, mv(ds), dz_in, dframe, dz_accumulate=dz_acc,
+            pend = nw.ipa_bwd(P, G, f"score_model.trunk.ipa_{b}", st["ipa"], dm, mv(ds), dz_in, dframe, dz_accumulate=dz_acc,
                               defer_dz=defer)
         _frame_grad_fold(st["bb"]["quat"], dframe, dq_in, dt_in, R)
         dq, dt, dnode, dz = dq_in, dt_in, ds, dz_in
         if not (defer_dw and b > 0 and sv["stages"][b - 1]["et"] is not None):
             ops.flush_dw()
         notify(b)
-    ops.add_view(mv(dnode), mv(dinit), R, CS)
     with rng("embed.bwd"):
-        nw.embed_bwd(P, G, sv["embed"], dnode, dz)
+        nw.embed_bwd(P, G, sv["embed"], dnode, dz, dnode2=dinit)
     ops.flush_dw()
     notify("embed")
     ops.join_grad_stream()
 
 
 def _frame_grad_fold(quat, dframe, dq, dt, R):
-    dev = quat
-    z4 = zeros((R, 4), dev); z3 = zeros((R, 3), dev); z6 = zeros((R, 6), dev); zm = zeros((R,), dev)
-    dq2 = empty((R, 4), dev); dt2 = empty((R, 3), dev); j1 = empty((R, 6), dev); j2 = empty((R, 6), dev)
-    lib().call("fd_bb_update_bwd", z4, z3, dframe, zm, z6, quat, dq2, dt2, j1, j2, R)
-    ops.add_view(mv(dq), mv(dq2), R, 4)
-    ops.add_view(mv(dt), mv(dt2), R, 3)
+    lib().call("fd_frame_grad_fold", quat, dframe, dq, dt, R)
```

After: 181,900. No clear change (-0.1%).
